# syzhang092218-source/dgppo

Hardware: AMD Instinct MI355X
Metric: env-steps/sec whole node, LidarSpread n=8 4096 envs, 1/2/4/8 GPUs (higher is better)
Workload: dtype f32

## Files before the change

dgppo_amd/csrc/env_step.h:

```cpp
#pragma once
#include "common.h"

enum { MODE_STEP = 0, MODE_SENSE = 1, MODE_GRAPH = 2 };

struct StepArgs {
  dgppo_env_cfg cfg;
  const float* agent;
  const float* action;
  const float* goal;
  const float* obst;
  const float* hits;
  const float* ray_cos;
  const float* ray_sin;
  float* next_agent;
  float* next_hits;
  float* reward;
  float* cost;
  dgppo_graph_out g;
  int has_graph;
  int mode;
  uint32_t rcp_n, rcp_k, rcp_no, rcp_no4;
  int B;
  float thr2_comm, thr2_lidar;
};

template <int SD>
__device__ inline void state2feat(const float* s, float* f) {
  if constexpr (SD == 5) {
    f[0] = s[0];
    f[1] = s[1];
    f[2] = s[4] * s[2];
    f[3] = s[4] * s[3];
  } else {
    f[0] = s[0]; f[1] = s[1]; f[2] = s[2]; f[3] = s[3];
  }
}

__device__ inline float clip_action(float u) { return clampf_nan(u, -1.0f, 1.0f); }


template <int SD>
__device__ inline void step_state(const float* x, float u0, float u1, const dgppo_env_cfg& c, float y_limit, float* nx) {
  const float dt = c.dt, A = c.area_size;
  if constexpr (SD == 5) {
    const float theta = atan2f(x[3], x[2]);
    const float theta_next = theta + x[4] * u0 * dt * 10.0f;
    nx[0] = clampf_nan(x[0] + x[4] * cosf(theta) * dt, 0.0f, A);
    nx[1] = clampf_nan(x[1] + x[4] * sinf(theta) * dt, 0.0f, A);
    nx[2] = clampf_nan(cosf(theta_next), -1.0f, 1.0f);
    nx[3] = clampf_nan(sinf(theta_next), -1.0f, 1.0f);
    nx[SD - 1] = clampf_nan(x[SD - 1] + u1 * dt * 10.0f, -0.5f, 0.5f);
  } else {
    const float vl = c.vel_limit;
    nx[0] = clampf_nan(x[2] * dt + x[0], 0.0f, A);
    nx[1] = clampf_nan(x[3] * dt + x[1], 0.0f, y_limit);
    nx[2] = clampf_nan((u0 * 10.0f) * dt + x[2], -vl, vl);
    nx[3] = clampf_nan((u1 * 10.0f) * dt + x[3], -vl, vl);
  }
}

__device__ inline float cost_value(float m) { return (m <= 0.0f) ? m - 0.5f : m + 0.5f; }

__device__ inline float reward_from_sums(float s1, float s2, float s3, int ng, int n) {
  float r = 0.0f;
  r = r - (s1 / (float)ng) * 0.01f;
  r = r - (s2 / (float)ng) * 0.001f;
  r = r - (s3 / (float)n) * 0.0001f;
  return r;
}

__device__ inline float segment_alpha_literal(float det0, float na, float nb) {
  const float sgn = (det0 > 0.0f) ? 1.0f : ((det0 < 0.0f) ? -1.0f : det0);
  const float det = sgn * fminf(fmaxf(fabsf(det0), 1e-7f), 1e7f);
  const float aq = na / det, bq = nb / det;
  const float v = ((aq <= 1.0f) && (aq >= 0.0f) && (bq <= 1.0f) && (bq >= 0.0f)) ? 1.0f : 0.0f;
  return v * aq + (1.0f - v) * 1e6f;
}

__device__ inline bool rect_inside(const float* rec, float px, float py, float r) {
  float rel_x = px - rec[0];
  float rel_y = py - rec[1];
  float c = rec[5], s = rec[6];
  float rel_xx = fabsf(rel_x * c + rel_y * s) - rec[2] / 2.0f;
  float rel_yy = fabsf(rel_x * s - rel_y * c) - rec[3] / 2.0f;
  bool is_in_down = (rel_xx < r) && (rel_yy < 0.0f);
  bool is_in_up = (rel_xx < 0.0f) && (rel_yy < r);
  bool is_out_corner = (rel_xx > 0.0f) && (rel_yy > 0.0f);
  bool is_in_circle = sqrtf(rel_xx * rel_xx + rel_yy * rel_yy) < r;
  return is_in_down || is_in_up || (is_out_corner && is_in_circle);
}


__device__ inline void segment_consts(const float* rec, int m, float* out4) {
  const int mm = (m + 3) & 3;
  const float* P = rec + 8;
  out4[0] = P[2 * m];
  out4[1] = P[2 * m + 1];
  out4[2] = P[2 * mm] - P[2 * m];
  out4[3] = P[2 * mm + 1] - P[2 * m + 1];
}

__device__ inline float ray_min_alpha(float x1, float y1, float rc, float rs, float sr, const float* s_seg, int no) {
  const float x2 = x1 + rc * sr;
  const float y2 = y1 + rs * sr;
  const float dx12 = x1 - x2, dy12 = y1 - y2;
  float amin = 0.0f;
  for (int o = 0; o < no; ++o) {
    float ao = 0.0f;
#pragma unroll
    for (int m = 0; m < 4; ++m) {
      const float4 sg = reinterpret_cast<const float4*>(s_seg)[o * 4 + m];
      const float x3 = sg.x, y3 = sg.y, ex = sg.z, ey = sg.w;
      const float det0 = dx12 * ey - dy12 * ex;
      const float ax = x1 - x3, ay = y1 - y3;
      const float na = ey * ax - ex * ay;
      const float nb = (-dy12) * ax + dx12 * ay;
      float al;
      if (det0 != 0.0f && det0 == det0) {
        const float det = copysignf(fminf(fmaxf(fabsf(det0), 1e-7f), 1e7f), det0);
        const bool pos = det > 0.0f;
        const bool va = (na == 0.0f || (na > 0.0f) == pos) && (pos ? (na <= det) : (na >= det));
        const bool vb = (nb == 0.0f || (nb > 0.0f) == pos) && (pos ? (nb <= det) : (nb >= det));
        al = 1e6f;
        if (va && vb) al = na / det + 0.0f;
      } else {
        al = segment_alpha_literal(det0, na, nb);
      }
      ao = (m == 0) ? al : nanmin(ao, al);
    }
    amin = (o == 0) ? ao : nanmin(amin, ao);
  }
  return amin;
}

__device__ inline int ray_rank(const float* al, int R, int r) {
  const float ar = al[r];
  const bool nr = (ar != ar);
  int rank = 0;
  for (int j = 0; j < R; ++j) {
    const float aj = al[j];
    const bool nj = (aj != aj);
    bool less;
    if (nj || nr) less = (nj == nr) ? (j < r) : nr;
    else less = (aj < ar) || (aj == ar && j < r);
    rank += less ? 1 : 0;
  }
  return rank;
}

__device__ inline void ray_hit(float x1, float y1, float rc, float rs, float sr, float ar, float* out2) {
  const float x2 = x1 + rc * sr;
  const float y2 = y1 + rs * sr;
  out2[0] = x1 + (x2 - x1) * ar;
  out2[1] = y1 + (y2 - y1) * ar;
}


#define MISS_BITS 0x49742400u

bool lidar_wave_has_instance(const dgppo_env_cfg& c);
void launch_lidar_wave(const StepArgs& a, hipStream_t s);
```

dgppo_amd/csrc/env_step.hip:

```cpp
#include "env_step.h"

template <int SD>
__global__ void env_step_kernel(StepArgs a) {
  extern __shared__ float smem[];
  const dgppo_env_cfg& c = a.cfg;
  const int b = blockIdx.x;
  const int tid = threadIdx.x, nt = blockDim.x;
  const int n = c.n_agents, ng = c.n_goals, no = c.n_obs, R = c.n_rays, k = c.top_k;
  const bool lidar = cfg_is_lidar(c), spread = cfg_is_spread(c);
  const int ostride = lidar ? DGPPO_RECT_STRIDE : SD;
  const int n_on = cfg_obs_nodes(c);
  const int kk = lidar ? (no > 0 ? k : 0) : 0;
  constexpr int ND = SD + 3;

  float* s_seg = smem;
  float* s_agent = s_seg + (lidar ? no * 16 : 0);
  float* s_next = s_agent + n * SD;
  float* s_goal = s_next + n * SD;
  float* s_act = s_goal + ng * SD;
  float* s_obst = s_act + n * 2;
  float* s_hpre = s_obst + no * ostride;
  float* s_hnext = s_hpre + n * kk * 2;
  float* s_alpha = s_hnext + n * kk * 2;
  float* s_fa = s_alpha + (lidar ? n * R : 0);
// ... 540 lines not shown
        const int e3 = e - n_aa - n_ag;
        i = DIVK(e3);
        const float lx = s_next[i * SD] - s_hnext[e3 * 2], ly = s_next[i * SD + 1] - s_hnext[e3 * 2 + 1];
        f = make_float4(lx, ly, 0.0f, 0.0f);
        mask = sqrtf(lx * lx + ly * ly) < c.lidar_mask_radius;
        sender = 2 * n + e3;
      }
      edges[e] = f;
      recv[e] = mask ? i : pad;
      send[e] = mask ? sender : pad;
    }
    int32_t* nty = a.g.node_type + (size_t)b * N;
    for (int node = tid; node < N; node += nt) nty[node] = (node < n) ? 0 : ((node < 2 * n) ? 1 : ((node < pad) ? 2 : -1));
    if (tid == 0) { a.g.n_node[b] = N; a.g.n_edge[b] = E; }
  }
  LDS_BARRIER();
  {
    float* nodes = a.g.nodes + (size_t)b * N * ND;
    for (int idx = tid; idx < N * ND; idx += nt) nodes[idx] = s_outn[idx];
    float* states = a.g.states + (size_t)b * N * SD;
    for (int idx = tid; idx < N * SD; idx += nt) states[idx] = s_outs[idx];
  }
}
#undef DIVN
#undef DIVK
#undef DIVNO
#undef DIVNO4

static size_t lidar_smem_bytes(const dgppo_env_cfg& c) {
  const size_t n = c.n_agents, no = c.n_obs, R = 32, k = c.top_k, SD = c.state_dim, NR = n * R;
  const size_t N = 2 * n + n * k + 1;
  size_t w = no * 16 + n * no * 16 + NR + n * 8 + no * 16 + n * SD * 3 + n * 2 + n * k * 4 + (2 * n * n + n * k) + n * no + 2 * n +
             N * (SD + 3) + N * SD;
  return w * 4;
}

static size_t step_smem_bytes(const dgppo_env_cfg& c) {
  const int n = c.n_agents, ng = c.n_goals, no = c.n_obs, SD = c.state_dim;
  const bool lidar = cfg_is_lidar(c);
  const int kk = lidar ? (no > 0 ? c.top_k : 0) : 0;
  size_t fl = (lidar ? (size_t)no * 16 : 0) + (size_t)n * SD * 2 + (size_t)ng * SD + n * 2 + (size_t)no * cfg_obst_stride(c) + (size_t)n * kk * 4 +
              (lidar ? (size_t)n * c.n_rays : 0) + n * 4 + ng * 4 + 3 * (size_t)cfg_reward_goals(c) + 3 * n + (size_t)n * no +
              (size_t)n * n + (size_t)n * (kk > no ? kk : no) + (size_t)cfg_reward_goals(c) * n;
  return fl * sizeof(float);
}

static float sqrt_threshold(float c) {
  if (!(c > 0.0f)) return 0.0f;
  float s = c * c;
  while (s > 0.0f && sqrtf(s) >= c) s = nextafterf(s, 0.0f);
  while (!(sqrtf(s) >= c)) s = nextafterf(s, INFINITY);
  return s;
}

enum StepFamily { FAMILY_WAVE, FAMILY_LIDAR_WG, FAMILY_GENERIC };

static StepFamily step_family(const StepArgs& a) {
  const dgppo_env_cfg& c = a.cfg;
  const bool lidar32 = cfg_is_lidar(c) && cfg_is_base_kind(c) && c.n_obs > 0 && c.n_rays == 32;
  auto al16 = [](const void* p) { return p == nullptr || (((uintptr_t)p) & 15) == 0; };
  const bool aligned = al16(a.agent) && al16(a.goal) && al16(a.obst) && al16(a.hits) && al16(a.next_agent) &&
                       al16(a.next_hits) && al16(a.action) && (!a.has_graph || (al16(a.g.edges) && al16(a.g.states)));
  if (lidar32 && c.top_k == 8 && c.eye_offset >= c.comm_radius && aligned && lidar_wave_has_instance(c)) return FAMILY_WAVE;
  if (lidar32 && lidar_smem_bytes(c) <= 60 * 1024) return FAMILY_LIDAR_WG;
  return FAMILY_GENERIC;
}

static int32_t launch_step(const dgppo_env_cfg* cfg, int mode, const float* agent, const float* action, const float* goal,
                           const float* obst, const float* hits, const float* ray_cos, const float* ray_sin,
                           float* next_agent, float* next_hits, float* reward, float* cost, const dgppo_graph_out* gout,
                           int32_t B, void* stream) {
  int32_t rc = dgppo_validate_cfg(cfg);
  if (rc) return rc;
  if (mode == MODE_GRAPH) DGPPO_REFUSE_VMAS(cfg, "dgppo_graph_materialize", "dgppo_vmas_graph_materialize");
  else DGPPO_REFUSE_VMAS(cfg, "dgppo_env_step", "dgppo_vmas_step");
  DGPPO_REQUIRE(B >= 0, "B must be >= 0 (got %d)", B);
  if (B == 0) return 0;
  const bool lidar = cfg_is_lidar(*cfg);
  DGPPO_REQUIRE(agent && goal, "agent/goal must not be NULL");
  DGPPO_REQUIRE(cfg->n_obs == 0 || obst, "obst must not be NULL when n_obs > 0");
  if (mode == MODE_STEP) {
    DGPPO_REQUIRE(action && reward && cost && next_agent, "step needs action, reward, cost and next_agent");
    DGPPO_REQUIRE(!(lidar && cfg->n_obs > 0) || hits, "LiDAR step needs the hit points of the current graph");
  }
  if (mode != MODE_GRAPH && lidar && cfg->n_obs > 0) {
    DGPPO_REQUIRE(ray_cos && ray_sin, "LiDAR sensing needs the ray tables");
    DGPPO_REQUIRE(next_hits || gout, "LiDAR sensing needs next_hits or a graph output");
  }
  if (mode == MODE_GRAPH) {
    DGPPO_REQUIRE(gout, "materialize needs a graph output");
    DGPPO_REQUIRE(!(lidar && cfg->n_obs > 0) || hits, "materialize needs hits for LiDAR envs");
  }
  StepArgs a;
  a.cfg = *cfg;
  a.agent = agent; a.action = action; a.goal = goal; a.obst = obst; a.hits = hits;
  a.ray_cos = ray_cos; a.ray_sin = ray_sin;
  a.next_agent = next_agent; a.next_hits = next_hits; a.reward = reward; a.cost = cost;
  a.has_graph = 0;
  a.g = dgppo_graph_out{};
  if (gout) {
    DGPPO_REQUIRE(gout->nodes && gout->edges && gout->states && gout->receivers && gout->senders && gout->node_type &&
                      gout->n_node && gout->n_edge,
                  "graph output must have all eight pointers set");
    DGPPO_REQUIRE(((uintptr_t)gout->edges & 15) == 0, "graph edges must be 16-byte aligned");
    a.g = *gout;
    a.has_graph = 1;
  }
  a.mode = mode;
  a.B = B;
  a.rcp_n = fdiv_rcp(cfg->n_agents); a.rcp_k = fdiv_rcp(cfg->top_k); a.rcp_no = fdiv_rcp(cfg->n_obs);
  a.rcp_no4 = fdiv_rcp(4 * (cfg->n_obs > 0 ? cfg->n_obs : 1));
  a.thr2_comm = sqrt_threshold(cfg->comm_radius);
  a.thr2_lidar = sqrt_threshold(cfg->lidar_mask_radius);
  const size_t smem = step_smem_bytes(*cfg);
  DGPPO_REQUIRE(smem <= 64 * 1024, "env too large for the per-env LDS stage (%zu bytes)", smem);
  hipStream_t s = (hipStream_t)stream;
  switch (step_family(a)) {
    case FAMILY_WAVE:
      launch_lidar_wave(a, s);
      break;
    case FAMILY_LIDAR_WG: {
      const size_t fsmem = lidar_smem_bytes(*cfg);
      if (cfg->state_dim == 5) hipLaunchKernelGGL((lidar_step_kernel<5, false, 128>), dim3(B), dim3(128), fsmem, s, a);
      else if (cfg_is_spread(*cfg)) hipLaunchKernelGGL((lidar_step_kernel<4, true, 128>), dim3(B), dim3(128), fsmem, s, a);
      else hipLaunchKernelGGL((lidar_step_kernel<4, false, 128>), dim3(B), dim3(128), fsmem, s, a);
      break;
    }
    case FAMILY_GENERIC: {
      int work = cfg->n_agents * (lidar ? cfg->n_rays : 1);
      const int E = cfg_num_edges(*cfg);
      if (gout && E > work) work = E;
      int threads = ((work + 63) / 64) * 64;
      if (threads < 64) threads = 64;
      if (threads > 512) threads = 512;
      if (cfg->state_dim == 5) hipLaunchKernelGGL(env_step_kernel<5>, dim3(B), dim3(threads), smem, s, a);
      else hipLaunchKernelGGL(env_step_kernel<4>, dim3(B), dim3(threads), smem, s, a);
      break;
    }
  }
  DGPPO_LAUNCH_CHECK();
  return 0;
}

extern "C" int32_t dgppo_env_step(const dgppo_env_cfg* cfg, const float* agent, const float* action, const float* goal,
                                  const float* obst, const float* hits, const float* ray_cos, const float* ray_sin,
                                  float* next_agent, float* next_hits, float* reward, float* cost,
                                  const dgppo_graph_out* gout, int32_t B, void* stream) {
  if (!cfg) { dgppo_set_error("cfg is NULL"); return -1; }
  const int mode = action ? MODE_STEP : MODE_SENSE;
  return launch_step(cfg, mode, agent, action, goal, obst, hits, ray_cos, ray_sin, next_agent, next_hits, reward, cost,
                     gout, B, stream);
}

extern "C" int32_t dgppo_graph_materialize(const dgppo_env_cfg* cfg, const float* agent, const float* goal,
                                           const float* obst, const float* hits, const dgppo_graph_out* gout, int32_t B,
                                           void* stream) {
  if (!cfg) { dgppo_set_error("cfg is NULL"); return -1; }
  return launch_step(cfg, MODE_GRAPH, agent, nullptr, goal, obst, hits, nullptr, nullptr, nullptr, nullptr, nullptr, nullptr,
                     gout, B, stream);
}
```

dgppo_amd/csrc/env_wave.hip:

```cpp
#include "env_step.h"

#ifndef DGPPO_WAVE_WPE
#define DGPPO_WAVE_WPE 5
#endif
#ifndef DGPPO_WAVE_WPE_COMPACT
#define DGPPO_WAVE_WPE_COMPACT 6
#endif
#ifndef DGPPO_WAVE_UNROLL_O
#define DGPPO_WAVE_UNROLL_O 8
#endif
#ifndef DGPPO_WAVE_UNROLL_P3
#define DGPPO_WAVE_UNROLL_P3 1
#endif
#define DGPPO_PRAGMA_(x) _Pragma(#x)
#define DGPPO_PRAGMA(x) DGPPO_PRAGMA_(x)

namespace {

#define WSYNC() asm volatile("" ::: "memory")
#ifdef DGPPO_STAMPS
__device__ unsigned long long g_wstamps[64];
__device__ unsigned long long g_wspan[3 * 8192];
#define PHASE(name, idx) do { asm volatile("; PHASE " name ::: "memory"); \
    if (blockIdx.x == 0 && threadIdx.x == 0 && stamp_on) g_wstamps[idx] = __builtin_amdgcn_s_memtime(); } while (0)
#elif defined(DGPPO_PHASE_MARKS)
#define PHASE(name, idx) asm volatile("; PHASE " name)
#else
#define PHASE(name, idx) do { } while (0)
#endif

constexpr int ceil4(int x) { return (x + 3) / 4 * 4; }

template <int SD, bool SPREAD, int NA, int NO>
struct WC {
  static constexpr int K = 8, R = 32, ND = SD + 3;
  static constexpr int NR = NA * R, NIT = NR / 64;
  static constexpr int NHIT = NA * K;
  static constexpr int N = 2 * NA + NHIT + 1, PAD = N - 1;
  static constexpr int GS = SPREAD ? NA : 1;
  static constexpr int E = NA * (NA + GS + K);
  static constexpr int NPAIR = NA * NO;
  static constexpr int NFAR = (NPAIR + 63) / 64;
  static_assert(NA % 2 == 0 && NA >= 2 && NA <= 16, "wave kernel: even n_agents <= 16 (two agents share a wave iteration)");
  static_assert((NA & (NA - 1)) == 0 && NA >= 4, "wave kernel: n_agents must be a power of two >= 4 (DPP group reductions)");
  static_assert(NO >= 1 && NO * 4 <= 64, "wave kernel: 1 <= n_obs <= 16");
  static_assert((NA * SD) % 4 == 0, "agent / goal rows are staged as float4");
  static_assert(ceil4(3 * NA) <= NA * SD && 4 * NA + ceil4(NA * 2) <= NO * 16, "overlays exceed the staged input they reuse");
};

template <int SD, bool SPREAD, int NA, int NO, bool GRAPH>
struct alignas(16) WaveLds {
  using C = WC<SD, SPREAD, NA, NO>;
  float4 seg[NO * 4];
  float4 pc[NA * NO];
  float4 circ[NO];
  uint32_t alpha[NA * 32];
  uint32_t badm[ceil4(NA)];
  union {
    uint16_t items[NA * NO * 32];
    struct {
      uint32_t tk[NA * 32];
      uint32_t hcnt[ceil4(NA)];
      uint16_t hlist[NA * 32];
    };
  };
  float next[ceil4(NA * SD)];
  union {
    float agent[NA * SD];
    float red[ceil4(3 * NA)];
  };
  float goal[NA * SD];
  union {
    float obst[NO * 16];
    struct {
      float sq[4 * NA];
      float cost[ceil4(NA * 2)];
    };
  };
  float hits[NA * C::K * 2];
  float act[ceil4(NA * 2)];
  float fa[SD == 4 ? 4 : NA * 4];
  float fg[SD == 4 ? 4 : NA * 4];
  float ino[ceil4(NA * NO)];
  float nodes[GRAPH ? ceil4(C::N * C::ND) : 4];
};

__device__ inline float raw_min(float a, float b) { float r; asm("v_min_f32 %0, %1, %2" : "=v"(r) : "v"(a), "v"(b)); return r; }
__device__ inline float raw_max(float a, float b) { float r; asm("v_max_f32 %0, %1, %2" : "=v"(r) : "v"(a), "v"(b)); return r; }

__device__ inline bool rect_inside_r0(const float* rec, float px, float py) {
  const float rel_x = px - rec[0], rel_y = py - rec[1];
  const float cs = rec[5], sn = rec[6];
  const float rel_xx = fabsf(rel_x * cs + rel_y * sn) - rec[2] / 2.0f;
  const float rel_yy = fabsf(rel_x * sn - rel_y * cs) - rec[3] / 2.0f;
  return (rel_xx < 0.0f) && (rel_yy < 0.0f);
}

template <int CTRL>
__device__ inline float dpp(float x) {
  return __int_as_float(__builtin_amdgcn_update_dpp(0, __float_as_int(x), CTRL, 0xF, 0xF, false));
}
constexpr int DPP_XOR1 = 0xB1;
constexpr int DPP_XOR2 = 0x4E;
constexpr int DPP_HALF_MIRROR = 0x141;
constexpr int DPP_ROW_MIRROR = 0x140;

template <int G>
__device__ inline float group_min(float x) {
  if (__builtin_amdgcn_ballot_w64(x != x) == 0ull) {
    x = raw_min(x, dpp<DPP_XOR1>(x));
    x = raw_min(x, dpp<DPP_XOR2>(x));
    if constexpr (G >= 8) x = raw_min(x, dpp<DPP_HALF_MIRROR>(x));
    if constexpr (G >= 16) x = raw_min(x, dpp<DPP_ROW_MIRROR>(x));
  } else {
    x = nanmin(x, dpp<DPP_XOR1>(x));
    x = nanmin(x, dpp<DPP_XOR2>(x));
    if constexpr (G >= 8) x = nanmin(x, dpp<DPP_HALF_MIRROR>(x));
    if constexpr (G >= 16) x = nanmin(x, dpp<DPP_ROW_MIRROR>(x));
  }
  return x;
}

template <int SD, bool SPREAD, int NA, int NO, int WPB, int MODE, bool GRAPH>
__global__ void __launch_bounds__(WPB * 64) __attribute__((amdgpu_waves_per_eu(GRAPH ? DGPPO_WAVE_WPE : DGPPO_WAVE_WPE_COMPACT, 8))) lidar_wave_kernel(StepArgs a) {
  using C = WC<SD, SPREAD, NA, NO>;
  using LT = WaveLds<SD, SPREAD, NA, NO, GRAPH>;
  constexpr int K = C::K, ND = C::ND, N = C::N, PAD = C::PAD, NIT = C::NIT, GS = C::GS, E = C::E;
  extern __shared__ float4 smem4[];
  int lane = threadIdx.x & 63;
  const int wave = __builtin_amdgcn_readfirstlane((int)(threadIdx.x >> 6));
  LT& L = reinterpret_cast<LT*>(smem4)[wave];
#ifdef DGPPO_STAMPS
  const int gw = blockIdx.x * WPB + wave;
  if ((threadIdx.x & 63) == 0 && gw < 8192) g_wspan[3 * gw] = __builtin_amdgcn_s_memtime();
#endif
  const dgppo_env_cfg& c = a.cfg;
  constexpr bool do_dyn = (MODE == MODE_STEP);
  constexpr bool do_sense = (MODE != MODE_GRAPH);
  constexpr bool has_graph = GRAPH;
  const float sr = c.comm_radius;
  const int r = lane & 31;
  const int hi_half = lane >> 5;
  const float cr = do_sense ? a.ray_cos[r] : 0.0f, sn = do_sense ? a.ray_sin[r] : 0.0f;
  const uint32_t below = (1u << r) - 1u;

  constexpr int I_AG = NA * SD / 4, I_OB = NO * 4, I_HI = (MODE != MODE_SENSE) ? NA * K * 2 / 4 : 0,
                I_AC = (MODE == MODE_STEP) ? NA * 2 / 4 : 0;
  constexpr int IT = 2 * I_AG + I_OB + I_HI + I_AC, NSLOT = (IT + 63) / 64;
  static_assert(MODE != MODE_STEP || (NA * 2) % 4 == 0, "the action block is staged as float4");
  const char* gsrc[NSLOT];
  uint32_t gstride[NSLOT];
  float4 pf[NSLOT];
#pragma unroll
  for (int j = 0; j < NSLOT; ++j) {
    const int q = j * 64 + lane;
    const char* base = reinterpret_cast<const char*>(a.agent);
    uint32_t stride = NA * SD * 4;
    int q0 = 0;
    if (q >= I_AG) { base = reinterpret_cast<const char*>(a.goal); q0 = I_AG; }
    if (q >= 2 * I_AG) { base = reinterpret_cast<const char*>(a.obst); stride = NO * 64; q0 = 2 * I_AG; }
    if (I_HI > 0 && q >= 2 * I_AG + I_OB) { base = reinterpret_cast<const char*>(a.hits); stride = NA * K * 8; q0 = 2 * I_AG + I_OB; }
    if (I_AC > 0 && q >= 2 * I_AG + I_OB + I_HI) { base = reinterpret_cast<const char*>(a.action); stride = NA * 8; q0 = 2 * I_AG + I_OB + I_HI; }
    gsrc[j] = base + (q - q0) * 16;
    gstride[j] = stride;
  }
  {
    const int b0 = blockIdx.x * WPB + wave;
    if (b0 < a.B) {
#pragma unroll
      for (int j = 0; j < NSLOT; ++j)
        if (j * 64 + lane < IT) pf[j] = *reinterpret_cast<const float4*>(gsrc[j] + (size_t)b0 * gstride[j]);
    }
  }
  if (has_graph)
    for (int i = lane; i < ceil4(N * ND) / 4; i += 64) reinterpret_cast<float4*>(L.nodes)[i] = make_float4(0.0f, 0.0f, 0.0f, 0.0f);
  WSYNC();
  if (has_graph)
    for (int node = lane; node < PAD; node += 64)
      L.nodes[node * ND + ((node < NA) ? SD + 2 : ((node < 2 * NA) ? SD + 1 : SD))] = 1.0f;
  WSYNC();

  for (int b = blockIdx.x * WPB + wave; b < a.B; b += gridDim.x * WPB) {
    asm volatile("" : "+v"(lane));
#ifdef DGPPO_STAMPS
    const bool stamp_on = (b == 0);
    if ((threadIdx.x & 63) == 0 && gw < 8192 && b == gw) g_wspan[3 * gw + 1] = __builtin_amdgcn_s_memtime();
    if (blockIdx.x == 0 && threadIdx.x == 0 && stamp_on) g_wstamps[40] = __builtin_amdgcn_s_memrealtime();
#endif
    PHASE("P0_stage", 0);
#pragma unroll
    for (int j = 0; j < NSLOT; ++j)
      if (j * 64 + lane < IT) reinterpret_cast<float4*>(L.agent)[j * 64 + lane] = pf[j];
    {
      const int bn = b + gridDim.x * WPB;
      if (bn < a.B) {
#pragma unroll
        for (int j = 0; j < NSLOT; ++j)
          if (j * 64 + lane < IT) pf[j] = *reinterpret_cast<const float4*>(gsrc[j] + (size_t)bn * gstride[j]);
      }
    }
    WSYNC();
    PHASE("P1a_dyn_seg_circ", 1);
    float asq = 0.0f;
    if (lane < NA) {
      const int i = lane;
      const float* x = L.agent + i * SD;
      float nx[SD];
      if (do_dyn) {
        const float u0 = clip_action(L.act[i * 2]), u1 = clip_action(L.act[i * 2 + 1]);
        step_state<SD>(x, u0, u1, c, c.area_size, nx);
        asq = u0 * u0 + u1 * u1;
      } else {
#pragma unroll
        for (int d = 0; d < SD; ++d) nx[d] = x[d];
      }
#pragma unroll
      for (int d = 0; d < SD; ++d) L.next[i * SD + d] = nx[d];
      if constexpr (SD != 4) state2feat<SD>(nx, L.fa + i * 4);
    }
    if constexpr (SD != 4)
      if (lane >= 32 && lane < 32 + NA) state2feat<SD>(L.goal + (lane - 32) * SD, L.fg + (lane - 32) * 4);
    const float* fa_ptr = (SD == 4) ? L.next : L.fa;
    const float* fg_ptr = (SD == 4) ? L.goal : L.fg;
    uint32_t robust_bits = 0;
    if (do_sense) {
      if (lane < NO * 4) {
        const int o = lane >> 2, m = lane & 3, mm = (m + 3) & 3;
        const float* P = L.obst + o * 16 + 8;
        L.seg[lane] = make_float4(P[2 * m], P[2 * m + 1], P[2 * mm] - P[2 * m], P[2 * mm + 1] - P[2 * m + 1]);
      }
      if (lane < NO) {
        const float* P = L.obst + lane * 16 + 8;
        const float cx = ((P[0] + P[2]) + (P[4] + P[6])) * 0.25f, cy = ((P[1] + P[3]) + (P[5] + P[7])) * 0.25f;
        float h2 = 0.0f;
#pragma unroll
        for (int m = 0; m < 4; ++m) {
          const float dx = P[2 * m] - cx, dy = P[2 * m + 1] - cy;
          h2 = fmaxf(h2, dx * dx + dy * dy);
        }
        const float hm = sqrtf(h2) + 0.05f, thr = sr + hm;
        L.circ[lane] = make_float4(cx, cy, thr * thr, hm);
      }
#pragma unroll
      for (int o = 0; o < NO; ++o) {
        const int m = hi_half, mm = (m + 3) & 3;
        const float* P = L.obst + o * 16 + 8;
        const float ex = P[2 * mm] - P[2 * m], ey = P[2 * mm + 1] - P[2 * m + 1];
        const float cc = cr * ey - sn * ex;
        const bool weak = !(fabsf(cc) >= 4e-4f);
        if (__builtin_amdgcn_ballot_w64(weak) == 0ull) robust_bits |= (1u << o);
      }
    }
    WSYNC();
    PHASE("P1b_far_as", 2);
    uint64_t far[C::NFAR];
    if (do_sense) {
#pragma unroll
      for (int w = 0; w < C::NFAR; ++w) {
        const int q = w * 64 + lane;
        bool isfar = false;
        if (q < C::NPAIR) {
          const int i = q / NO, o = q - i * NO;
          const float px = L.next[i * SD], py = L.next[i * SD + 1];
          L.ino[q] = rect_inside_r0(L.obst + o * 16, px, py) ? 1.0f : 0.0f;
          const float4 cc = L.circ[o];
          const float dx = px - cc.x, dy = py - cc.y;
          const bool robust = (robust_bits >> o) & 1u;
          isfar = (dx * dx + dy * dy > cc.z) && robust;
          L.pc[q] = make_float4(cc.x - px, cc.y - py, isfar ? -1.0f : (robust ? cc.w : __builtin_inff()), 0.0f);
        }
        far[w] = __builtin_amdgcn_ballot_w64(isfar);
      }
    } else {
#pragma unroll
      for (int w = 0; w < C::NFAR; ++w) far[w] = 0ull;
    }
    PHASE("P1c_cost_terms", 3);
    if (do_dyn) {
      WSYNC();
      if (lane < NA) L.sq[3 * NA + lane] = asq;
    }
    if (do_dyn) {
#pragma unroll
      for (int q0 = 0; q0 < NA * NA; q0 += 64) {
        const int q = q0 + lane, i = q / NA, j = q - i * NA;
        float d = __builtin_inff();
        if (q < NA * NA && j != i) {
          const float dx = L.agent[i * SD] - L.agent[j * SD], dy = L.agent[i * SD + 1] - L.agent[j * SD + 1];
          d = dx * dx + dy * dy;
        }
        const float md2 = group_min<NA>(d);
        if (q < NA * NA && j == 0) L.sq[i] = md2;
      }
#pragma unroll
      for (int q0 = 0; q0 < NA * K; q0 += 64) {
        const int q = q0 + lane, i = q / K;
        float d = __builtin_inff();
        if (q < NA * K) {
          const float dx = L.hits[q * 2] - L.agent[i * SD], dy = L.hits[q * 2 + 1] - L.agent[i * SD + 1];
          d = dx * dx + dy * dy;
        }
        const float mo2 = group_min<K>(d);
        if (q < NA * K && (q & (K - 1)) == 0) L.sq[NA + i] = mo2;
      }
      if constexpr (SPREAD) {
#pragma unroll
        for (int q0 = 0; q0 < NA * NA; q0 += 64) {
          const int q = q0 + lane, g = q / NA, j = q - g * NA;
          float d = __builtin_inff();
          if (q < NA * NA) {
            const float dx = L.goal[g * SD] - L.agent[j * SD], dy = L.goal[g * SD + 1] - L.agent[j * SD + 1];
            d = dx * dx + dy * dy;
          }
          const float g2 = group_min<NA>(d);
          if (q < NA * NA && j == 0) L.sq[2 * NA + g] = g2;
        }
      } else {
        if (lane < NA) {
          const int g = lane;
          const float dx = L.goal[g * SD] - L.agent[g * SD], dy = L.goal[g * SD + 1] - L.agent[g * SD + 1];
          L.sq[2 * NA + g] = dx * dx + dy * dy;
        }
      }
      WSYNC();
      static_assert(4 * NA <= 64, "one lane per pending square root");
      if (lane < 4 * NA) {
        const float rt = sqrtf(L.sq[lane]);
        const int kind = lane / NA, i = lane - kind * NA;
        if (kind == 0) {
          const float md = nanmin(rt, 1e6f);
          L.cost[i * 2] = clampf_nan(cost_value(c.two_car_radius - md), -1.0f, 1.0f);
        } else if (kind == 1) {
          L.cost[i * 2 + 1] = clampf_nan(cost_value(c.car_radius - rt), -1.0f, 1.0f);
        } else if (kind == 2) {
          L.red[i] = rt;
          L.red[NA + i] = (rt > c.dist2goal) ? 1.0f : 0.0f;
        } else {
          L.red[2 * NA + i] = rt * rt;
        }
      }
    }
    WSYNC();
    PHASE("P1d_reward", 4);
    if (do_dyn) {
      float s = 0.0f;
      if (lane < 3) {
        s = L.red[lane * NA];
#pragma unroll
        for (int g = 1; g < NA; ++g) s = s + L.red[lane * NA + g];
      }
      const float s1 = __int_as_float(__builtin_amdgcn_readlane(__float_as_int(s), 0));
      const float s2 = __int_as_float(__builtin_amdgcn_readlane(__float_as_int(s), 1));
      const float s3 = __int_as_float(__builtin_amdgcn_readlane(__float_as_int(s), 2));
      if (lane == 0) a.reward[b] = reward_from_sums(s1, s2, s3, NA, NA);
      if (lane < NA * 2) a.cost[(size_t)b * NA * 2 + lane] = L.cost[lane];
    }
    if (a.next_agent != nullptr) {
      float4* o4 = reinterpret_cast<float4*>(a.next_agent + (size_t)b * NA * SD);
      for (int i = lane; i < NA * SD / 4; i += 64) o4[i] = reinterpret_cast<const float4*>(L.next)[i];
    }
    if (has_graph) {
      for (int q = lane; q < NA * SD; q += 64) {
        const int node = q / SD, d = q - node * SD;
        const float va = L.next[q], vg = L.goal[q];
        L.nodes[node * ND + d] = va;
        L.nodes[(NA + node) * ND + d] = vg;
      }
    }
    if (has_graph) {
      float4* edges = reinterpret_cast<float4*>(a.g.edges) + (size_t)b * E;
      int32_t* recv = a.g.receivers + (size_t)b * E;
      int32_t* send = a.g.senders + (size_t)b * E;
#pragma unroll
      for (int q0 = 0; q0 < NA * NA; q0 += 64) {
        const int q = q0 + lane;
        if (q < NA * NA) {
          const int i = q / NA, j = q - i * NA;
          const float4 fi = reinterpret_cast<const float4*>(fa_ptr)[i], fj = reinterpret_cast<const float4*>(fa_ptr)[j];
          const float dx = L.next[i * SD] - L.next[j * SD], dy = L.next[i * SD + 1] - L.next[j * SD + 1];
          const bool mask = (i != j) && (dx * dx + dy * dy < a.thr2_comm);
          edges[q] = make_float4(fi.x - fj.x, fi.y - fj.y, fi.z - fj.z, fi.w - fj.w);
          recv[q] = mask ? i : PAD;
          send[q] = mask ? j : PAD;
        }
      }
#pragma unroll
      for (int q0 = 0; q0 < NA * GS; q0 += 64) {
        const int q = q0 + lane;
        if (q < NA * GS) {
          const int i = SPREAD ? q / NA : q, g = SPREAD ? q - i * NA : q;
          const float4 fi = reinterpret_cast<const float4*>(fa_ptr)[i], fg = reinterpret_cast<const float4*>(fg_ptr)[g];
          edges[NA * NA + q] = make_float4(fi.x - fg.x, fi.y - fg.y, fi.z - fg.z, fi.w - fg.w);
          recv[NA * NA + q] = i;
          send[NA * NA + q] = NA + g;
        }
      }
      int32_t* nty = a.g.node_type + (size_t)b * N;
#pragma unroll
      for (int q0 = 0; q0 < N; q0 += 64) {
        const int node = q0 + lane;
        if (node < N) nty[node] = (node < NA) ? 0 : ((node < 2 * NA) ? 1 : ((node < PAD) ? 2 : -1));
      }
      if (lane == 0) { a.g.n_node[b] = N; a.g.n_edge[b] = E; }
    }
    PHASE("P2_rays", 5);
    if (do_sense) {
      for (int q = lane; q < NA * 32 / 4; q += 64)
        reinterpret_cast<uint4*>(L.alpha)[q] = make_uint4(MISS_BITS, MISS_BITS, MISS_BITS, MISS_BITS);
      if (lane < ceil4(NA)) L.badm[lane] = 0u;
      int total = 0;
      constexpr int GSTEPS = (2 * NO * NIT <= 32) ? NIT : ((32 / (2 * NO)) >= 1 ? (32 / (2 * NO)) : 1);
      static_assert(2 * NO <= 32, "one step's triples must fit the lane mask");
#pragma unroll
      for (int g0 = 0; g0 < NIT; g0 += GSTEPS) {
        uint32_t nmask = 0u;
#pragma unroll
        for (int it = g0; it < g0 + GSTEPS && it < NIT; ++it) {
#pragma unroll
          for (int o = 0; o < NO; ++o) {
            const int qa = (it * 2) * NO + o, qb = (it * 2 + 1) * NO + o;
            const bool fa_ = (far[qa >> 6] >> (qa & 63)) & 1ull, fb_ = (far[qb >> 6] >> (qb & 63)) & 1ull;
            if (fa_ && fb_) continue;
            const float4 pc = L.pc[(it * 2 + hi_half) * NO + o];
            const float cross = cr * pc.y - sn * pc.x, dot = cr * pc.x + sn * pc.y;
            const bool need = !(fabsf(cross) > pc.z) && !(dot < -pc.z);
            nmask |= need ? (1u << ((it - g0) * 2 * NO + o)) : 0u;
          }
        }
        const int cnt = __popc(nmask);
        int inc = cnt;
        inc += __builtin_amdgcn_update_dpp(0, inc, 0x111, 0xF, 0xF, false);
        inc += __builtin_amdgcn_update_dpp(0, inc, 0x112, 0xF, 0xF, false);
        inc += __builtin_amdgcn_update_dpp(0, inc, 0x114, 0xF, 0xF, false);
        inc += __builtin_amdgcn_update_dpp(0, inc, 0x118, 0xF, 0xF, false);
        inc += __builtin_amdgcn_update_dpp(0, inc, 0x142, 0xA, 0xF, false);
        inc += __builtin_amdgcn_update_dpp(0, inc, 0x143, 0xC, 0xF, false);
        int pos = total + inc - cnt;
        total += __builtin_amdgcn_readlane(inc, 63);
        const uint32_t base_code = ((uint32_t)((2 * g0 + hi_half) * NO) << 5) | (uint32_t)r;
        while (__builtin_amdgcn_ballot_w64(nmask != 0u) != 0ull) {
          if (nmask != 0u) {
            const int bit = __builtin_ctz(nmask);
            L.items[pos] = (uint16_t)(base_code + ((uint32_t)bit << 5));
            pos += 1;
            nmask &= nmask - 1u;
          }
        }
      }
      WSYNC();
      PHASE("P2b_dense", 6);
#pragma unroll 1
      for (int k0 = 0; k0 < total; k0 += 64) {
        const int k = k0 + lane;
        const uint32_t item = L.items[k < total ? k : 0];
        const int rr = (int)(item & 31u);
        const float crr = __int_as_float(__builtin_amdgcn_ds_bpermute(rr << 2, __float_as_int(cr)));
        const float snr = __int_as_float(__builtin_amdgcn_ds_bpermute(rr << 2, __float_as_int(sn)));
        if (k < total) {
          const int pair = (int)(item >> 5);
          const int i = pair / NO, o = pair - i * NO;
          const float x1 = L.next[i * SD], y1 = L.next[i * SD + 1];
          const float x2 = x1 + crr * sr, y2 = y1 + snr * sr;
          const float dx12 = x1 - x2, dy12 = y1 - y2, ndy12 = -dy12;
          float naf[4], adet[4];
          bool valid[4];
          float dprod = 1.0f;
#pragma unroll
          for (int m = 0; m < 4; ++m) {
            const float4 sg = L.seg[o * 4 + m];
            const float ax = x1 - sg.x, ay = y1 - sg.y;
            const float na = sg.w * ax - sg.z * ay;
            const float det0 = dx12 * sg.w - dy12 * sg.z;
            const float nb = ndy12 * ax + dx12 * ay;
            const uint32_t sb = __float_as_uint(det0) & 0x80000000u;
            naf[m] = __uint_as_float(__float_as_uint(na) ^ sb);
            const float nbf = __uint_as_float(__float_as_uint(nb) ^ sb);
            adet[m] = __builtin_amdgcn_fmed3f(fabsf(det0), 1e-7f, 1e7f);
            const float mn = raw_min(naf[m], nbf), mx = raw_max(naf[m], nbf);
            valid[m] = (mn >= 0.0f) && (mx <= adet[m]);
            dprod = dprod * det0;
          }
          const bool bad = !(fabsf(dprod) > 0.0f);
          float amin = 1e6f;
          if (__builtin_amdgcn_ballot_w64(valid[0] || valid[1] || valid[2] || valid[3]) != 0ull) {
#pragma unroll
            for (int m = 0; m < 4; ++m) {
              const float qa_ = naf[m] / adet[m] + 0.0f;
              const float al = valid[m] ? qa_ : 1e6f;
              amin = raw_min(amin, al);
            }
          }
          if (amin < 1e6f) atomicMin(&L.alpha[i * 32 + rr], __float_as_uint(amin));
          if (bad) atomicOr(&L.badm[i], 1u << rr);
        }
      }
      WSYNC();
      PHASE("P2_slowcheck", 10);
      if (__builtin_amdgcn_ballot_w64(lane < NA && L.badm[lane < NA ? lane : 0] != 0u) != 0ull) {
#pragma unroll 1
        for (int it = 0; it < NIT; ++it) {
          const int i = it * 2 + hi_half;
          if ((L.badm[i] >> r) & 1u) {
            const float x1 = L.next[i * SD], y1 = L.next[i * SD + 1];
            const float x2 = x1 + cr * sr, y2 = y1 + sn * sr;
            const float dx12 = x1 - x2, dy12 = y1 - y2, ndy12 = -dy12;
            float lmin = 1e6f;
            bool any_nan = false;
#pragma unroll 1
            for (int q = 0; q < NO * 4; ++q) {
              const float4 sgq = L.seg[q];
              const float ax = x1 - sgq.x, ay = y1 - sgq.y;
              const float na = sgq.w * ax - sgq.z * ay;
// ... 58 lines not shown
          const int rr = (int)(rec & 31u);
          const float crr = __int_as_float(__builtin_amdgcn_ds_bpermute(rr << 2, __float_as_int(cr)));
          const float snr = __int_as_float(__builtin_amdgcn_ds_bpermute(rr << 2, __float_as_int(sn)));
          if (k < n_hits) {
            const int i = (int)(rec >> 10), p = (int)((rec >> 5) & 31u);
            const uint32_t kr = L.tk[i * 32 + p];
            int rank = 0;
#pragma unroll 1
            for (int cb = 0; cb < cmaxw; cb += 4) {
              const uint4 ks = *reinterpret_cast<const uint4*>(&L.tk[i * 32 + cb]);
              rank += ((ks.x < kr) || (ks.x == kr && cb + 0 < p)) ? 1 : 0;
              rank += ((ks.y < kr) || (ks.y == kr && cb + 1 < p)) ? 1 : 0;
              rank += ((ks.z < kr) || (ks.z == kr && cb + 2 < p)) ? 1 : 0;
              rank += ((ks.w < kr) || (ks.w == kr && cb + 3 < p)) ? 1 : 0;
            }
            if (rank < K) {
              const float x1 = L.next[i * SD], y1 = L.next[i * SD + 1];
              const float x2 = x1 + crr * sr, y2 = y1 + snr * sr;
              const float ar = __uint_as_float(kr);
              const float hx = x1 + (x2 - x1) * ar, hy = y1 + (y2 - y1) * ar;
              const int hq = i * K + rank, node = 2 * NA + hq;
              L.hits[hq * 2] = hx; L.hits[hq * 2 + 1] = hy;
              if (has_graph) { L.nodes[node * ND] = hx; L.nodes[node * ND + 1] = hy; }
            }
          }
        }
      } else {
        WSYNC();
  #pragma unroll 1
        for (int it = 0; it < NIT; ++it) {
          const int i = it * 2 + hi_half;
          const float x1 = L.next[i * SD], y1 = L.next[i * SD + 1];
          const float x2 = x1 + cr * sr, y2 = y1 + sn * sr;
          float is_in = 0.0f;
  #pragma unroll
          for (int o = 0; o < NO; ++o) is_in = fmaxf(is_in, L.ino[i * NO + o]);
          float ar = __uint_as_float(L.alpha[i * 32 + r]);
          ar = ar * (1.0f - is_in);
          PHASE("P3_topk", 12 + it * 3 + 1);
          int rank;
          if (__builtin_amdgcn_ballot_w64(ar != ar) == 0ull) {
            const uint32_t kr = __float_as_uint(ar);
            const bool hit = kr < MISS_BITS;
            const uint64_t Lm = __builtin_amdgcn_ballot_w64(hit);
            const uint32_t lo = (uint32_t)Lm, hi = (uint32_t)(Lm >> 32);
            const int n_lo = __popc(lo), n_hi = __popc(hi);
            const int p = (int)__builtin_amdgcn_mbcnt_hi(hi, __builtin_amdgcn_mbcnt_lo(lo, 0u)) - (hi_half ? n_lo : 0);
            const bool allz = is_in != 0.0f;
            const bool z_lo = __builtin_amdgcn_readlane((int)allz, 0) != 0, z_hi = __builtin_amdgcn_readlane((int)allz, 32) != 0;
            const int c_lo = z_lo ? 0 : n_lo, c_hi = z_hi ? 0 : n_hi;
            const int cmax = c_lo > c_hi ? c_lo : c_hi;
            rank = allz ? r : ((hi_half ? n_hi : n_lo) + r - p);
            if (cmax > 0) {
              const bool isL = hit && !allz;
              L.tk[lane] = 0xFFFFFFFFu;
              WSYNC();
              if (isL) L.tk[hi_half * 32 + p] = kr;
              WSYNC();
              int rlt = 0;
  #pragma unroll 1
              for (int cb = 0; cb < cmax; cb += 4) {
                const uint4 ks = *reinterpret_cast<const uint4*>(&L.tk[hi_half * 32 + cb]);
                rlt += (ks.x < kr ? 1 : 0) + (ks.y < kr ? 1 : 0) + (ks.z < kr ? 1 : 0) + (ks.w < kr ? 1 : 0);
              }
              WSYNC();
              if (isL) L.tk[hi_half * 32 + rlt] = (uint32_t)p;
              WSYNC();
              const bool lost = isL && (L.tk[hi_half * 32 + rlt] != (uint32_t)p);
              if (__builtin_amdgcn_ballot_w64(lost) != 0ull) {
                WSYNC();
                L.tk[lane] = 0xFFFFFFFFu;
                WSYNC();
                if (isL) L.tk[hi_half * 32 + p] = kr;
                WSYNC();
                rlt = 0;
  #pragma unroll 1
                for (int sl = 0; sl < cmax; ++sl) {
                  const uint32_t kj = L.tk[hi_half * 32 + sl];
                  rlt += (kj < kr || (kj == kr && sl < p)) ? 1 : 0;
                }
                WSYNC();
              }
              if (isL) rank = rlt;
            }
          } else {
            const uint32_t kr = (ar != ar) ? 0xFFFFFFFFu : __float_as_uint(ar);
            const uint64_t Lm = __builtin_amdgcn_ballot_w64(kr < MISS_BITS);
            const uint64_t Mm = __builtin_amdgcn_ballot_w64(kr == MISS_BITS);
            const uint64_t Zm = __builtin_amdgcn_ballot_w64(kr == 0u);
            const uint32_t lo = (uint32_t)Lm, hi = (uint32_t)(Lm >> 32);
            const uint32_t myL = hi_half ? hi : lo;
            const uint32_t myM = hi_half ? (uint32_t)(Mm >> 32) : (uint32_t)Mm;
            const int cntL = __popc(myL);
            const int rank_other = (kr == MISS_BITS) ? cntL + __popc(myM & below)
                                                     : cntL + __popc(myM) + __popc(~(myL | myM) & below);
            const bool z_lo = ((uint32_t)Zm == 0xFFFFFFFFu), z_hi = ((uint32_t)(Zm >> 32) == 0xFFFFFFFFu);
            const bool allz = hi_half ? z_hi : z_lo;
            const bool isL = (kr < MISS_BITS) && !allz;
            const int p = __popc(myL & below);
            L.tk[lane] = 0xFFFFFFFFu;
            WSYNC();
            if (isL) L.tk[hi_half * 32 + p] = kr;
            WSYNC();
            const int c_lo = z_lo ? 0 : __popc(lo), c_hi = z_hi ? 0 : __popc(hi);
            const int cmax = c_lo > c_hi ? c_lo : c_hi;
            int rlt = 0;
    #pragma unroll 1
            for (int cb = 0; cb < cmax; cb += 4) {
              const uint4 ks = *reinterpret_cast<const uint4*>(&L.tk[hi_half * 32 + cb]);
              rlt += (ks.x < kr ? 1 : 0) + (ks.y < kr ? 1 : 0) + (ks.z < kr ? 1 : 0) + (ks.w < kr ? 1 : 0);
            }
            WSYNC();
            if (isL) L.tk[hi_half * 32 + rlt] = (uint32_t)p;
            WSYNC();
            const bool lost = isL && (L.tk[hi_half * 32 + rlt] != (uint32_t)p);
            if (__builtin_amdgcn_ballot_w64(lost) != 0ull) {
              WSYNC();
              L.tk[lane] = 0xFFFFFFFFu;
              WSYNC();
              if (isL) L.tk[hi_half * 32 + p] = kr;
              WSYNC();
              rlt = 0;
    #pragma unroll 1
              for (int sl = 0; sl < cmax; ++sl) {
                const uint32_t kj = L.tk[hi_half * 32 + sl];
                rlt += (kj < kr || (kj == kr && sl < p)) ? 1 : 0;
              }
              WSYNC();
            }
            rank = allz ? r : (isL ? rlt : rank_other);
          }
          if (rank < K) {
            const float hx = x1 + (x2 - x1) * ar, hy = y1 + (y2 - y1) * ar;
            const int hq = i * K + rank, node = 2 * NA + hq;
            L.hits[hq * 2] = hx; L.hits[hq * 2 + 1] = hy;
            if (has_graph) { L.nodes[node * ND] = hx; L.nodes[node * ND + 1] = hy; }
          }
          PHASE("P3_end", 12 + it * 3 + 2);
        }
      }
    } else {
      for (int q = lane; q < NA * K; q += 64) {
        const float hx = L.hits[q * 2], hy = L.hits[q * 2 + 1];
        const int node = 2 * NA + q;
        if (has_graph) { L.nodes[node * ND] = hx; L.nodes[node * ND + 1] = hy; }
      }
    }
    WSYNC();
    PHASE("P4_compact", 7);
    if (a.next_hits != nullptr) {
      float4* o4 = reinterpret_cast<float4*>(a.next_hits + (size_t)b * NA * K * 2);
      for (int i = lane; i < NA * K * 2 / 4; i += 64) o4[i] = reinterpret_cast<const float4*>(L.hits)[i];
    }
    if (!has_graph) continue;
    PHASE("P5_graph", 8);
    {
      float4* edges = reinterpret_cast<float4*>(a.g.edges) + (size_t)b * E;
      int32_t* recv = a.g.receivers + (size_t)b * E;
      int32_t* send = a.g.senders + (size_t)b * E;
#pragma unroll
      for (int q0 = 0; q0 < NA * K; q0 += 64) {
        const int q = q0 + lane;
        if (q < NA * K) {
          const int i = q / K;
          const float lx = L.next[i * SD] - L.hits[q * 2], ly = L.next[i * SD + 1] - L.hits[q * 2 + 1];
          const bool mask = lx * lx + ly * ly < a.thr2_lidar;
          edges[NA * NA + NA * GS + q] = make_float4(lx, ly, 0.0f, 0.0f);
          recv[NA * NA + NA * GS + q] = mask ? i : PAD;
          send[NA * NA + NA * GS + q] = mask ? 2 * NA + q : PAD;
        }
      }
      float* nodes = a.g.nodes + (size_t)b * N * ND;
#pragma unroll
      for (int q0 = 0; q0 < N * ND; q0 += 64) {
        const int q = q0 + lane;
        if (q < N * ND) nodes[q] = L.nodes[q];
      }
      if constexpr (SD == 4) {
        float4* st4 = reinterpret_cast<float4*>(a.g.states + (size_t)b * N * SD);
#pragma unroll
        for (int q0 = 0; q0 < N; q0 += 64) {
          const int node = q0 + lane;
          if (node < N) {
            const float* row = L.nodes + node * ND;
            st4[node] = (node == PAD) ? make_float4(-1.0f, -1.0f, -1.0f, -1.0f) : make_float4(row[0], row[1], row[2], row[3]);
          }
        }
      } else {
        float* st = a.g.states + (size_t)b * N * SD;
#pragma unroll
        for (int q0 = 0; q0 < N * SD; q0 += 64) {
          const int q = q0 + lane;
          if (q < N * SD) {
            const int node = q / SD, d = q - node * SD;
            st[q] = (node == PAD) ? -1.0f : L.nodes[node * ND + d];
          }
        }
      }
    }
    WSYNC();
    PHASE("env_end", 9);
#ifdef DGPPO_STAMPS
    if (blockIdx.x == 0 && threadIdx.x == 0 && stamp_on) g_wstamps[41] = __builtin_amdgcn_s_memrealtime();
    if ((threadIdx.x & 63) == 0 && gw < 8192) g_wspan[3 * gw + 2] = __builtin_amdgcn_s_memtime();
#endif
  }
}

template <int SD, bool SPREAD, int NA, int NO>
void launch_inst(const StepArgs& a, hipStream_t s) {
  constexpr size_t per_wave = sizeof(WaveLds<SD, SPREAD, NA, NO, true>);
  constexpr int WPB = (per_wave * 4 <= 40 * 1024) ? 4 : ((per_wave * 2 <= 52 * 1024) ? 2 : 1);
  static_assert(per_wave * WPB <= 64 * 1024, "LDS slab too large");
  constexpr size_t smem_g = per_wave * WPB, smem_c = sizeof(WaveLds<SD, SPREAD, NA, NO, false>) * WPB;
  static int per_cu_cached[3][2] = {{0, 0}, {0, 0}, {0, 0}};
  int& per_cu = per_cu_cached[a.mode][a.has_graph ? 1 : 0];
  if (per_cu == 0) {
    int n = 0;
    hipError_t e = hipErrorUnknown;
#define OCC(M_, G_) e = hipOccupancyMaxActiveBlocksPerMultiprocessor(&n, lidar_wave_kernel<SD, SPREAD, NA, NO, WPB, M_, G_>, WPB * 64, (G_) ? smem_g : smem_c)
    if (a.mode == MODE_STEP) { if (a.has_graph) OCC(MODE_STEP, true); else OCC(MODE_STEP, false); }
    else if (a.mode == MODE_SENSE) { if (a.has_graph) OCC(MODE_SENSE, true); else OCC(MODE_SENSE, false); }
    else OCC(MODE_GRAPH, true);
#undef OCC
    per_cu = (e == hipSuccess && n > 0) ? n : 1;
  }
  int n_cu = 256;
  {
    static int cached_cu = 0;
    if (cached_cu == 0) {
      int dev = 0, v = 0;
      if (hipGetDevice(&dev) == hipSuccess && hipDeviceGetAttribute(&v, hipDeviceAttributeMultiprocessorCount, dev) == hipSuccess && v > 0)
        cached_cu = v;
      else
        cached_cu = 256;
    }
    n_cu = cached_cu;
  }
  const int max_blocks = n_cu * per_cu;
  int blocks = (a.B + WPB - 1) / WPB;
  if (blocks > max_blocks) blocks = max_blocks;
  const dim3 g(blocks), t(WPB * 64);
#define LAUNCH(M_, G_) hipLaunchKernelGGL((lidar_wave_kernel<SD, SPREAD, NA, NO, WPB, M_, G_>), g, t, (G_) ? smem_g : smem_c, s, a)
  if (a.mode == MODE_STEP) { if (a.has_graph) LAUNCH(MODE_STEP, true); else LAUNCH(MODE_STEP, false); }
  else if (a.mode == MODE_SENSE) { if (a.has_graph) LAUNCH(MODE_SENSE, true); else LAUNCH(MODE_SENSE, false); }
  else LAUNCH(MODE_GRAPH, true);
#undef LAUNCH
}

template <int SD_, bool SPREAD_, int NA_, int NO_>
struct Inst { static constexpr int SD = SD_, NA = NA_, NO = NO_; static constexpr bool SPREAD = SPREAD_; };

template <class F>
bool with_instance(const dgppo_env_cfg& c, F&& f) {
  const bool spread = cfg_is_spread(c);
  const int n = c.n_agents, no = c.n_obs, sd = c.state_dim;
#define INST(SD_, SP_, NA_, NO_) if (sd == SD_ && spread == SP_ && n == NA_ && no == NO_) { f(Inst<SD_, SP_, NA_, NO_>{}); return true; }
  INST(4, true, 8, 3);
  INST(4, false, 8, 3);
  INST(5, false, 16, 8);
  INST(4, true, 16, 8);
  INST(4, true, 4, 2);
  INST(4, false, 4, 2);
  INST(5, false, 4, 3);
#undef INST
  return false;
}

}

#ifdef DGPPO_STAMPS
extern "C" int32_t dgppo_debug_wave_stamps(unsigned long long* out) {
  return (int32_t)hipMemcpyFromSymbol(out, HIP_SYMBOL(g_wstamps), sizeof(unsigned long long) * 64);
}
extern "C" int32_t dgppo_debug_wave_spans(unsigned long long* out) {
  return (int32_t)hipMemcpyFromSymbol(out, HIP_SYMBOL(g_wspan), sizeof(unsigned long long) * 3 * 8192);
}
#endif

bool lidar_wave_has_instance(const dgppo_env_cfg& c) { return with_instance(c, [](auto) {}); }

void launch_lidar_wave(const StepArgs& a, hipStream_t s) {
  with_instance(a.cfg, [&](auto inst) {
    using I = decltype(inst);
    launch_inst<I::SD, I::SPREAD, I::NA, I::NO>(a, s);
  });
}
```

dgppo_amd/csrc/nn_elem.hip:

```cpp
#include "common.h"
#include "nn_ln.h"
#include "nn_gru.h"

using f32x4 = __attribute__((ext_vector_type(4))) float;

__device__ inline float wave_sum(float v) {
#pragma unroll
  for (int o = 32; o >= 1; o >>= 1) v += __shfl_xor(v, o);
  return v;
}
template <int NV>
__device__ inline void block_atomic_sums(const float (&v)[NV], float* dst) {
  __shared__ float s_red[4][NV];
  const int lane = threadIdx.x & 63, wave = threadIdx.x >> 6;
#pragma unroll
  for (int k = 0; k < NV; ++k) {
    const float w = wave_sum(v[k]);
    if (lane == 0) s_red[wave][k] = w;
  }
  __syncthreads();
  if (threadIdx.x < NV) {
    float t = 0.0f;
    for (int w = 0; w < (int)(blockDim.x >> 6); ++w) t += s_red[w][threadIdx.x];
    atomicAdd(dst + threadIdx.x, t);
// ... 322 lines not shown
      for (int rt = 0; rt < RTW; ++rt)
#pragma unroll
        for (int r = 0; r < 4; ++r) {
          const int rl = rt * 16 + lq * 4 + r;
          const float d = ok[rt][r] ? dh[rt][r] + du[rt][r] : 0.0f;
          const GruGateGrad gg = gru_gate_grad(d, hp[rt][r], rg[rt][r], zg[rt][r], ng[rt][r], hn[rt][r]);
          const float dar = gg.dar, daz = gg.daz, dan = gg.dan, dhn = gg.dhn;
          dh[rt][r] = d * zg[rt][r];
          if (tau > 0) {
            s_g[rl * GRU_WL + c] = dar;
            s_g[rl * GRU_WL + 64 + c] = daz;
            s_g[rl * GRU_WL + 128 + c] = dhn;
          }
          if (ok[rt][r]) {
            const size_t row = (size_t)(row0[rt][r] + tau * a.n_inner);
            float* o = a.dgi + row * 192 + c;
            o[0] = dar; o[64] = daz; o[128] = dan;
            if (DHN_ONLY) {
              a.dhn[row * GRU_H + c] = dhn;
            } else {
              float* p = a.dgh + row * 192 + c;
              p[0] = dar; p[64] = daz; p[128] = dhn;
            }
          }
        }
      if (tau == 0) break;
      GRU_LDS_BARRIER();
      fetch(tau - 1);
      __builtin_amdgcn_sched_barrier(0);
      f32x4 acc[RTW];
#pragma unroll
      for (int rt = 0; rt < RTW; ++rt) acc[rt] = f32x4{0.f, 0.f, 0.f, 0.f};
#pragma unroll
      for (int k0 = 0; k0 < 48; k0 += 16) {
        float areg[RTW][16];
#pragma unroll
        for (int rt = 0; rt < RTW; ++rt)
#pragma unroll
          for (int u = 0; u < 16; ++u) areg[rt][u] = s_g[(rt * 16 + li) * GRU_WL + (k0 + u) * 4 + lq];
        __builtin_amdgcn_sched_barrier(0);
#pragma unroll
        for (int u = 0; u < 16; ++u)
#pragma unroll
          for (int rt = 0; rt < RTW; ++rt) acc[rt] = __builtin_amdgcn_mfma_f32_16x16x4f32(areg[rt][u], breg[k0 + u], acc[rt], 0, 0, 0);
      }
#pragma unroll
      for (int rt = 0; rt < RTW; ++rt)
#pragma unroll
        for (int r = 0; r < 4; ++r) dh[rt][r] += acc[rt][r];
      cur ^= 1;
    }
    GRU_LDS_BARRIER();
  }
}

static int gru_resident(const void* fn, size_t smem) {
  int per_cu = 0, dev = 0, cus = 256;
  if (hipOccupancyMaxActiveBlocksPerMultiprocessor(&per_cu, fn, 256, smem) != hipSuccess || per_cu < 1) per_cu = 1;
  if (hipGetDevice(&dev) != hipSuccess ||
      hipDeviceGetAttribute(&cus, hipDeviceAttributeMultiprocessorCount, dev) != hipSuccess || cus < 1) cus = 256;
  return per_cu * cus;
}

static int32_t gru_check(const GruArgs& a) {
  DGPPO_REQUIRE(a.n_seq >= 0 && a.T >= 1 && a.n_inner >= 1, "gru: bad sizes n_seq=%d T=%d n_inner=%d", a.n_seq, a.T, a.n_inner);
  DGPPO_REQUIRE(a.n_seq % a.n_inner == 0, "gru: n_seq must be a multiple of n_inner");
  return 0;
}

static int32_t gru_fwd_launch(GruArgs a, hipStream_t stream) {
  int32_t rc = gru_check(a);
  if (rc) return rc;
  const int n_seq = a.n_seq;
  if (n_seq == 0) return 0;
  DGPPO_REQUIRE(a.gi && a.Wh && a.bhn && a.hs, "gru_fwd: NULL operand");
  if (cdiv(n_seq, 32) >= 512) {
    const size_t smem = sizeof(float) * 2 * 32 * GRU_HL;
    static thread_local int cap = 0;
    if (cap == 0) cap = gru_resident(reinterpret_cast<const void*>(&gru_fwd_kernel<2>), smem);
    const int tiles = cdiv(n_seq, 32);
    hipLaunchKernelGGL(gru_fwd_kernel<2>, dim3(tiles < cap ? tiles : cap), dim3(256), smem, stream, a);
  } else {
    const size_t smem = sizeof(float) * 2 * 16 * GRU_HL;
    static thread_local int cap = 0;
    if (cap == 0) cap = gru_resident(reinterpret_cast<const void*>(&gru_fwd_kernel<1>), smem);
    const int tiles = cdiv(n_seq, 16);
    hipLaunchKernelGGL(gru_fwd_kernel<1>, dim3(tiles < cap ? tiles : cap), dim3(256), smem, stream, a);
  }
  DGPPO_LAUNCH_CHECK();
  return 0;
}

extern "C" int32_t dgppo_gru_fwd(const float* gi, const float* Wh, const float* bhn, const float* h0, float* hs,
                                 float* hprev, float* gates, int32_t n_seq, int32_t T, int32_t n_inner, void* stream) {
  GruArgs a{};
  a.gi = gi; a.Wh = Wh; a.bhn = bhn; a.h0 = h0; a.hs = hs; a.hprev = hprev; a.gates = gates;
  a.n_seq = n_seq; a.T = T; a.n_inner = n_inner;
  return gru_fwd_launch(a, (hipStream_t)stream);
}

extern "C" int32_t dgppo_gru_fwd_h0_blocks(const float* gi, const float* Wh, const float* bhn, const float* h0,
                                           int32_t rows_per_block, int64_t block_stride, float* hs, float* hprev,
                                           float* gates, int32_t n_seq, int32_t T, int32_t n_inner, void* stream) {
  GruArgs a{};
  a.gi = gi; a.Wh = Wh; a.bhn = bhn; a.h0 = h0; a.hs = hs; a.hprev = hprev; a.gates = gates;
  a.n_seq = n_seq; a.T = T; a.n_inner = n_inner;
  DGPPO_REQUIRE(h0 != nullptr && ((uintptr_t)h0 & 15) == 0, "gru_fwd_h0_blocks: h0 must be a 16-byte aligned pointer");
  DGPPO_REQUIRE(rows_per_block >= 1, "gru_fwd_h0_blocks: rows_per_block must be >= 1 (got %d)", rows_per_block);
  DGPPO_REQUIRE(block_stride >= (int64_t)rows_per_block * GRU_H && block_stride % 4 == 0,
                "gru_fwd_h0_blocks: block_stride must be a multiple of 4 and >= rows_per_block * 64");
  a.h0_rpb = rows_per_block; a.h0_bstride = (long)block_stride;
  return gru_fwd_launch(a, (hipStream_t)stream);
}

template <bool DHN_ONLY>
static int32_t gru_bwd_launch(GruArgs a, hipStream_t stream) {
  int32_t rc = gru_check(a);
  if (rc) return rc;
  if (a.n_seq == 0) return 0;
  DGPPO_REQUIRE(a.dhs && a.Wh && a.hprev && a.gates && a.dgi && (DHN_ONLY ? a.dhn : a.dgh), "gru_bwd: NULL operand");
  if (cdiv(a.n_seq, 32) >= 512) {
    const size_t smem = sizeof(float) * 2 * 32 * GRU_WL;
    static thread_local int cap = 0;
    if (cap == 0) cap = gru_resident(reinterpret_cast<const void*>(&gru_bwd_kernel<2, DHN_ONLY>), smem);
    const int tiles = cdiv(a.n_seq, 32);
    hipLaunchKernelGGL((gru_bwd_kernel<2, DHN_ONLY>), dim3(tiles < cap ? tiles : cap), dim3(256), smem, stream, a);
  } else {
    const size_t smem = sizeof(float) * 2 * 16 * GRU_WL;
    static thread_local int cap = 0;
    if (cap == 0) cap = gru_resident(reinterpret_cast<const void*>(&gru_bwd_kernel<1, DHN_ONLY>), smem);
    const int tiles = cdiv(a.n_seq, 16);
    hipLaunchKernelGGL((gru_bwd_kernel<1, DHN_ONLY>), dim3(tiles < cap ? tiles : cap), dim3(256), smem, stream, a);
  }
  DGPPO_LAUNCH_CHECK();
  return 0;
}

extern "C" int32_t dgppo_gru_bwd(const float* dhs, const float* Wh, const float* hprev, const float* gates, float* dgi,
                                 float* dgh, int32_t n_seq, int32_t T, int32_t n_inner, void* stream) {
  GruArgs a{};
  a.dhs = dhs; a.Wh = Wh; a.hprev = (float*)hprev; a.gates = (float*)gates; a.dgi = dgi; a.dgh = dgh;
  a.n_seq = n_seq; a.T = T; a.n_inner = n_inner;
  return gru_bwd_launch<false>(a, (hipStream_t)stream);
}

extern "C" int32_t dgppo_gru_bwd_dhn(const float* dhs, const float* Wh, const float* hprev, const float* gates, float* dgi,
                                     float* dhn, int32_t n_seq, int32_t T, int32_t n_inner, void* stream) {
  GruArgs a{};
  a.dhs = dhs; a.Wh = Wh; a.hprev = (float*)hprev; a.gates = (float*)gates; a.dgi = dgi; a.dhn = dhn;
  a.n_seq = n_seq; a.T = T; a.n_inner = n_inner;
  return gru_bwd_launch<true>(a, (hipStream_t)stream);
}

#define STD_INIT_INV (-0.43275212956718856f)
#define STD_MIN 1e-5f
#define THRESH 0.999f
#define INV_THRESH 3.8002011672502f
#define LOG_EPS (-6.907755278982137f)
#define HALF_LOG_2PI 0.9189385332046727f
#define LOG2_F 0.6931471805599453f

__device__ inline float softplusf_(float x) { return (x > 20.0f) ? x : log1pf(expf(x)); }
#define NDTR_SERIES_BELOW (-10.0f)
__device__ inline float ndtr_tail_series(float z2) { return 1.0f - 1.0f / z2 + 3.0f / (z2 * z2) - 15.0f / (z2 * z2 * z2); }
__device__ inline float log_ndtrf_(float z) {
  if (z > NDTR_SERIES_BELOW) return logf(0.5f * erfcf(-z * 0.70710678118654752f));
  const float z2 = z * z;
  return -0.5f * z2 - logf(-z) - HALF_LOG_2PI + logf(ndtr_tail_series(z2));
}
__device__ inline float dlog_ndtrf_(float z) {
  if (z > NDTR_SERIES_BELOW) return 0.3989422804014327f * expf(-0.5f * z * z) / (0.5f * erfcf(-z * 0.70710678118654752f));
  return -z / ndtr_tail_series(z * z);
}
__device__ inline float tanh_fldj(float x) { return 2.0f * (LOG2_F - x - softplusf_(-2.0f * x)); }

struct HeadArgs {
  const float* ms;
  const float* eps;
  const float* action_in;
  float* action;
  float* log_pi;
  float* entropy;
  int rows, n_agents, mode;
  const float* log_pi_old;
  const float* adv;
  float* dms;
  float* stats;
  float clip_eps, coef_ent, inv_count;
};

__device__ inline float tn_log_prob_dim(float act, float mu, float sd) {
  const float ac = fminf(fmaxf(act, -THRESH), THRESH);
  if (ac <= -THRESH) return log_ndtrf_((-INV_THRESH - mu) / sd) - LOG_EPS;
  if (ac >= THRESH) return log_ndtrf_(-(INV_THRESH - mu) / sd) - LOG_EPS;
  const float x = atanhf(ac);
  const float z = (x - mu) / sd;
  return -0.5f * z * z - logf(sd) - HALF_LOG_2PI - tanh_fldj(x);
}

__global__ void __launch_bounds__(256) policy_head_kernel(HeadArgs a) {
  float acc[4] = {0.0f, 0.0f, 0.0f, 0.0f};
  const int rows_pad = (a.rows + 255) & ~255;
  for (int row_raw = blockIdx.x * blockDim.x + threadIdx.x; row_raw < rows_pad; row_raw += gridDim.x * blockDim.x) {
  const bool valid = row_raw < a.rows;
  const int row = valid ? row_raw : a.rows - 1;
  const float4 m = reinterpret_cast<const float4*>(a.ms)[row];
  const float mu[2] = {m.x, m.y};
  const float st[2] = {m.z, m.w};
  float sd[2];
  for (int d = 0; d < 2; ++d) sd[d] = softplusf_(st[d] + STD_INIT_INV) + STD_MIN;
  if (a.mode == 1) {
    if (valid) {
      a.action[row * 2] = tanhf(mu[0]);
      a.action[row * 2 + 1] = tanhf(mu[1]);
    }
    continue;
  }
  float act[2];
  if (a.mode == 0) {
    for (int d = 0; d < 2; ++d) act[d] = tanhf(mu[d] + sd[d] * a.eps[row * 2 + d]);
    if (valid) {
      a.action[row * 2] = act[0];
      a.action[row * 2 + 1] = act[1];
      a.log_pi[row] = tn_log_prob_dim(act[0], mu[0], sd[0]) + tn_log_prob_dim(act[1], mu[1], sd[1]);
    }
    continue;
  }
  act[0] = a.action_in[row * 2];
  act[1] = a.action_in[row * 2 + 1];
  const int ag = row % a.n_agents;
  float lp = 0.0f, ent = 0.0f;
  float dlp_dmu[2], dlp_dsd[2], dent_dmu[2], dent_dsd[2];
  for (int d = 0; d < 2; ++d) {
    const float ac = fminf(fmaxf(act[d], -THRESH), THRESH);
    if (ac <= -THRESH) {
      const float u = (-INV_THRESH - mu[d]) / sd[d];
      lp += log_ndtrf_(u) - LOG_EPS;
      const float r = dlog_ndtrf_(u);
      dlp_dmu[d] = -r / sd[d];
      dlp_dsd[d] = -r * u / sd[d];
    } else if (ac >= THRESH) {
      const float u = (mu[d] - INV_THRESH) / sd[d];
      lp += log_ndtrf_(u) - LOG_EPS;
      const float r = dlog_ndtrf_(u);
      dlp_dmu[d] = r / sd[d];
      dlp_dsd[d] = -r * u / sd[d];
    } else {
      const float x = atanhf(ac);
      const float z = (x - mu[d]) / sd[d];
      lp += -0.5f * z * z - logf(sd[d]) - HALF_LOG_2PI - tanh_fldj(x);
      dlp_dmu[d] = z / sd[d];
      dlp_dsd[d] = (z * z - 1.0f) / sd[d];
    }
    const float eh = a.eps[ag * 2 + d];
    const float y = mu[d] + sd[d] * eh;
    ent += 0.5f + HALF_LOG_2PI + logf(sd[d]) + tanh_fldj(y);
    const float th = tanhf(y);
    dent_dmu[d] = -2.0f * th;
    dent_dsd[d] = 1.0f / sd[d] - 2.0f * th * eh;
  }
  if (valid) {
    a.log_pi[row] = lp;
    a.entropy[row] = ent;
  }
  if (a.dms == nullptr) continue;
  const float A = a.adv[row];
  const float rho = expf(lp - a.log_pi_old[row]);
  const float l1 = -rho * A;
  const float l2 = -fminf(fmaxf(rho, 1.0f - a.clip_eps), 1.0f + a.clip_eps) * A;
  const float lsel = fmaxf(l1, l2);
  const float dl_dlp = ((l2 > l1) ? 0.0f : -rho * A) * a.inv_count;
  const float dl_dent = -a.coef_ent * a.inv_count;
  if (valid) {
    float4 o;
    const float dsd0 = dl_dlp * dlp_dsd[0] + dl_dent * dent_dsd[0];
    const float dsd1 = dl_dlp * dlp_dsd[1] + dl_dent * dent_dsd[1];
    o.x = dl_dlp * dlp_dmu[0] + dl_dent * dent_dmu[0];
    o.y = dl_dlp * dlp_dmu[1] + dl_dent * dent_dmu[1];
    o.z = dsd0 * sigmoidf_(st[0] + STD_INIT_INV);
    o.w = dsd1 * sigmoidf_(st[1] + STD_INIT_INV);
    reinterpret_cast<float4*>(a.dms)[row] = o;
  }
  if (valid) {
    acc[0] += lsel; acc[1] += ent; acc[2] += (l2 > l1) ? 1.0f : 0.0f; acc[3] += fabsf(rho - 1.0f);
  }
  }
  if (a.mode == 2 && a.dms != nullptr) block_atomic_sums<4>(acc, a.stats);
}

extern "C" int32_t dgppo_policy_head(const float* ms, const float* eps, const float* action_in, float* action,
                                     float* log_pi, float* entropy, int32_t rows, int32_t n_agents, int32_t mode,
                                     const float* log_pi_old, const float* adv, float* dms, float* stats, float clip_eps,
                                     float coef_ent, void* stream) {
  DGPPO_REQUIRE(rows >= 0 && n_agents >= 1 && mode >= 0 && mode <= 2, "policy_head: bad arguments");
  if (rows == 0) return 0;
  DGPPO_REQUIRE(ms, "policy_head: ms is NULL");
  DGPPO_REQUIRE(((uintptr_t)ms & 15) == 0, "policy_head: ms must be 16-byte aligned");
  if (mode == 0) DGPPO_REQUIRE(eps && action && log_pi, "policy_head(sample): NULL operand");
  if (mode == 1) DGPPO_REQUIRE(action, "policy_head(mode): NULL operand");
  if (mode == 2) {
    DGPPO_REQUIRE(eps && action_in && log_pi && entropy, "policy_head(eval): NULL operand");
    if (dms) DGPPO_REQUIRE(log_pi_old && adv && stats && ((uintptr_t)dms & 15) == 0, "policy_head(eval+loss): NULL operand");
  }
  HeadArgs a{};
  a.ms = ms; a.eps = eps; a.action_in = action_in; a.action = action; a.log_pi = log_pi; a.entropy = entropy;
  a.rows = rows; a.n_agents = n_agents; a.mode = mode; a.log_pi_old = log_pi_old; a.adv = adv; a.dms = dms; a.stats = stats;
  a.clip_eps = clip_eps; a.coef_ent = coef_ent; a.inv_count = 1.0f / (float)rows;
  const int blocks = cdiv(rows, 256);
  hipLaunchKernelGGL(policy_head_kernel, dim3(blocks < 512 ? blocks : 512), dim3(256), 0, (hipStream_t)stream, a);
  DGPPO_LAUNCH_CHECK();
  return 0;
}

__global__ void __launch_bounds__(256) value_loss_kernel(const float* __restrict__ v, const float* __restrict__ target,
                                                         float* __restrict__ dv, float* __restrict__ stats, int count,
                                                         float count_f) {
  float l[1] = {0.0f};
  for (int i = blockIdx.x * blockDim.x + threadIdx.x; i < count; i += gridDim.x * blockDim.x) {
    const float d = v[i] - target[i];
    dv[i] = d / count_f;
    l[0] += 0.5f * d * d;
  }
  block_atomic_sums<1>(l, stats);
}

extern "C" int32_t dgppo_value_loss(const float* v, const float* target, float* dv, float* stats, int32_t count,
                                    void* stream) {
  DGPPO_REQUIRE(count >= 0, "value_loss: count < 0");
  if (count == 0) return 0;
  DGPPO_REQUIRE(v && target && dv && stats, "value_loss: NULL operand");
  const int blocks = cdiv(count, 256);
  hipLaunchKernelGGL(value_loss_kernel, dim3(blocks < 256 ? blocks : 256), dim3(256), 0, (hipStream_t)stream, v, target, dv,
                     stats, count, (float)count);
  DGPPO_LAUNCH_CHECK();
  return 0;
}

__global__ void mean_agents_kernel(const float* __restrict__ x, float* __restrict__ y, int G, int n, int D, int backward,
                                   const float* __restrict__ relu_mask) {
  const int idx = blockIdx.x * blockDim.x + threadIdx.x;
  if (backward) {
    if (idx >= G * n * D) return;
    const int d = idx % D, g = idx / (n * D);
    const float v = (backward == 2) ? y[idx] + x[(size_t)g * D + d] : x[(size_t)g * D + d] / (float)n;
    y[idx] = (relu_mask == nullptr || relu_mask[idx] > 0.0f) ? v : 0.0f;
  } else {
    if (idx >= G * D) return;
    const int d = idx % D, g = idx / D;
    float acc = 0.0f;
    for (int i = 0; i < n; ++i) acc += x[((size_t)g * n + i) * D + d];
    y[idx] = acc / (float)n;
  }
}

extern "C" int32_t dgppo_mean_agents(const float* x, float* y, int32_t G, int32_t n, int32_t D, int32_t backward,
                                     const float* relu_mask, void* stream) {
  DGPPO_REQUIRE(G >= 0 && n >= 1 && D >= 1, "mean_agents: bad sizes");
  DGPPO_REQUIRE(backward >= 0 && backward <= 2, "mean_agents: backward must be 0, 1 or 2");
  if (G == 0) return 0;
  DGPPO_REQUIRE(x && y, "mean_agents: NULL operand");
  const long total = backward ? (long)G * n * D : (long)G * D;
  hipLaunchKernelGGL(mean_agents_kernel, dim3(cdiv(total, 256)), dim3(256), 0, (hipStream_t)stream, x, y, G, n, D, backward,
                     backward ? relu_mask : nullptr);
  DGPPO_LAUNCH_CHECK();
  return 0;
}

__global__ void relu_bwd_kernel(float* __restrict__ dy, const float* __restrict__ y, long count) {
  const long i = (long)blockIdx.x * blockDim.x + threadIdx.x;
  if (i < count && !(y[i] > 0.0f)) dy[i] = 0.0f;
}

extern "C" int32_t dgppo_relu_bwd(float* dy, const float* y, int64_t count, void* stream) {
// ... 8 lines not shown
```

dgppo_amd/engine.py:

```python
from __future__ import annotations

import dataclasses
from typing import Callable, Dict, Optional

import numpy as np
import os
import torch

from . import _native as N
from . import nets
from . import ops_algo as OA
from . import ops_env as OE
from . import ops_nn as K
from .utils import checkpoint as CK


@dataclasses.dataclass
class Hyper:
    gamma: float = 0.99
    gae_lambda: float = 0.95
    clip_eps: float = 0.25
    coef_ent: float = 1e-2
    max_grad_norm: float = 2.0
    lr_actor: float = 3e-4
    lr_Vl: float = 1e-3
    lr_Vh: float = 1e-3
    batch_size: int = 16384
    rnn_step: int = 16
    alpha: float = 10.0
    cbf_eps: float = 1e-2
    cbf_weight: float = 1.0
    cbf_schedule: bool = True
    train_steps: int = 100000
    actor_gnn_layers: int = 2
    Vl_gnn_layers: int = 2
    Vh_gnn_layers: int = 1
    use_rnn: bool = True
    use_lstm: bool = False
    rnn_layers: int = 1
    lagr_init: float = 0.78
    lr_lagr: float = 1e-7
    cost_weight: float = 0.0
    cost_schedule: bool = False


class RolloutData:

    def __init__(self, cfg: N.EnvCfg, B: int, T: int, device, stochastic: bool, carry_dim: int = nets.HID):
        n = cfg.n_agents
        self.cfg, self.B, self.T, self.stochastic = cfg, B, T, stochastic
        z = lambda *s: torch.empty(*s, device=device)
        step, env = OE.record_fields(cfg)
        self.step_tm = {k: z(T + 1, B, *shape) for k, shape in step.items()}
        self.env = {k: z(B, *shape) for k, shape in env.items()}
        self.step: Dict[str, torch.Tensor] = {}
        for k in OE.STEP_FIELDS:
            setattr(self, k + "_tm", self.step_tm.get(k))
            setattr(self, k, None)
        for k in OE.ENV_FIELDS:
            setattr(self, k, self.env.get(k))
        self.action_tm = z(T, B, n, 2)
        self.log_pi_tm = z(T, B, n) if stochastic else None
        self.rnn_tm = z(T + 1, B, n, carry_dim)
        self.reward_tm = z(T, B)
        self.cost_tm = z(T, B, n, cfg.n_cost)
        self._env_major = False
        views = {k: v.unbind(0) for k, v in self.step_tm.items()}
        self.states_tm = [OE.State({k: v[t] for k, v in views.items()}, self.env) for t in range(T + 1)]

    def finalize(self):
        if self._env_major:
            return self

        def tr(name, x):
            if x is None:
                return None
            cur = getattr(self, name, None)
            want = (x.shape[1], x.shape[0]) + tuple(x.shape[2:])
            if cur is None or tuple(cur.shape) != want:
                cur = torch.empty(want, device=x.device, dtype=x.dtype)
            cur.copy_(x.transpose(0, 1))
            return cur
        for k, v in self.step_tm.items():
            self.step[k] = tr(k, v)
            setattr(self, k, self.step[k])
        self.actions = tr("actions", self.action_tm)
        self.log_pis = tr("log_pis", self.log_pi_tm) if self.stochastic else None
        T, x = self.T, self.rnn_tm
        want = (x.shape[1], T + 2) + tuple(x.shape[2:])
        cur = getattr(self, "_rnn_em", None)
        if cur is None or tuple(cur.shape) != want:
            cur = torch.empty(want, device=x.device, dtype=x.dtype)
        cur[:, :T + 1].copy_(x.transpose(0, 1))
        self._rnn_em = cur
        self.rnn_states = self._rnn_em[:, :T] if self.stochastic else self._rnn_em[:, 1:T + 1]
        self.rewards = tr("rewards", self.reward_tm)
        self.costs = tr("costs", self.cost_tm)
        self._env_major = True
        return self


class OptState:
    def __init__(self, n: int, device):
        self.m = torch.zeros(n, device=device)
        self.v = torch.zeros(n, device=device)
        self.state = torch.zeros(N.OPT_STATE_FLOATS, device=device)


class Engine:
    def __init__(self, cfg: N.EnvCfg, hyper: Hyper, device, T: int = 128,
                 allreduce: Optional[Callable[[torch.Tensor], None]] = None, world: int = 1, prepass_graphs: int = 1 << 20,
                 use_graphs: bool = False, multi_stream: bool = False, algo: str = "dgppo", rank: int = 0):
        self.cfg, self.hp, self.device, self.T = cfg, hyper, device, T
        assert algo in ("dgppo", "informarl", "hcbfcrpo", "informarl_lagr"), algo
        self.algo = algo
        self.use_graphs = use_graphs and os.environ.get("DGPPO_HIPGRAPH", "1") != "0"
        self.multi_stream = multi_stream and os.environ.get("DGPPO_MULTI_STREAM", "1") != "0"
        self._side_streams = None
        self._ro_cache: Dict[tuple, dict] = {}
        self._upd_graph: dict = {}
        self.n_cost = cfg.n_cost
        spec = [("policy", "policy", hyper.actor_gnn_layers, 2), ("Vl", "Vl", hyper.Vl_gnn_layers, 1)]
        if algo == "dgppo":
            spec.append(("Vh", "Vh", hyper.Vh_gnn_layers, self.n_cost))
        elif algo == "informarl_lagr":
            spec.append(("Vh", "Vhg", hyper.Vh_gnn_layers, self.n_cost))
        def rnn_kw(name):
            if not hyper.use_rnn:
                return dict(rnn="none", rnn_layers=0)
            if name == "Vh" and algo == "dgppo":
                return dict(rnn="gru", rnn_layers=1)
            return dict(rnn="lstm" if hyper.use_lstm else "gru", rnn_layers=hyper.rnn_layers)
        sizes = [nets.make_layout(kind, cfg.node_dim, layers, n_out, **rnn_kw(k)).size for k, kind, layers, n_out in spec]
        offs, tot = [], 0
        for sz in sizes:
            offs.append(tot)
            tot += (sz + 3) // 4 * 4
        self.flat_grads = torch.zeros(tot + 4 * 8, device=device)
        self.n_reduced = tot + 3 * 8
        self.stats = self.flat_grads[tot:tot + 32].view(4, 8)
        built = {k: nets.Net(kind, cfg, layers, n_out, device, grads=self.flat_grads[o:o + sz], **rnn_kw(k))
                 for (k, kind, layers, n_out), o, sz in zip(spec, offs, sizes)}
        if algo == "informarl_lagr":
            self.lagr = torch.full((cfg.n_agents, self.n_cost), float(hyper.lagr_init), device=device)
            self.lagr_sums = torch.zeros(cfg.n_agents * self.n_cost, device=device)
        self.policy, self.Vl, self.Vh = built["policy"], built["Vl"], built.get("Vh")
        self.HC = self.policy.carry_dim
        self.opt = {k: OptState(net.layout.size, device) for k, net in self.nets.items()}
        self.arena = nets.Arena(device)
        self.allreduce = allreduce
        self.world, self.rank = int(world), int(rank)
        assert self.world >= 1 and (allreduce is not None or self.world == 1), "world > 1 needs an allreduce"
        assert 0 <= self.rank < self.world, f"rank {rank} outside world {world}"
        self.prepass_graphs = int(os.environ.get("DGPPO_PREPASS_GRAPHS", prepass_graphs))
        self.lam_pow = OA.lam_pow_table(hyper.gae_lambda, T, device)
        self.eps_hat = torch.zeros(cfg.n_agents, 2, device=device)
        self.reset_failed = torch.zeros(1, dtype=torch.int32, device=device)
        self.grad_hook: Optional[Callable[[str, nets.Net, int], None]] = None
        self._mb = 0

    @property
    def nets(self) -> Dict[str, nets.Net]:
        d = {"policy": self.policy, "Vl": self.Vl}
        if self.Vh is not None:
            d["Vh"] = self.Vh
        return d

    def set_entropy_noise(self, seed: int):
        OE.randn(seed, 0, self.eps_hat.view(-1))

    _CFG_IDENTITY = ("kind", "n_agents", "n_obs", "n_rays", "top_k", "node_dim", "n_cost")

    def _identity(self) -> dict:
        ident = {"algo": CK.encode_str(self.algo)}
        ident.update({f"cfg.{k}": int(getattr(self.cfg, k)) for k in self._CFG_IDENTITY})
        for f in dataclasses.fields(Hyper):
            v = getattr(self.hp, f.name)
            ident[f"hyper.{f.name}"] = int(v) if isinstance(v, (bool, int)) else float(v)
        ident["T"], ident["world"] = int(self.T), int(self.world)
        ident.update({f"size.{k}": int(net.layout.size) for k, net in self.nets.items()})
        return ident

    def _state_tensors(self) -> Dict[str, torch.Tensor]:
        t = {}
        for k, net in self.nets.items():
            opt = self.opt[k]
            t.update({f"{k}/params": net.params, f"{k}/m": opt.m, f"{k}/v": opt.v, f"{k}/state": opt.state})
        t["eps_hat"] = self.eps_hat
        if self.algo == "informarl_lagr":
            t["lagr"] = self.lagr
        return t

    def state_dict(self) -> dict:
        out = {"identity": self._identity()}
        for path, x in self._state_tensors().items():
            node = out
            *dirs, leaf = path.split("/")
            for d in dirs:
                node = node.setdefault(d, {})
            node[leaf] = x.detach().cpu().numpy().copy()
        return out

    def load_state_dict(self, d: dict) -> None:
        mine, theirs = self._identity(), d.get("identity", {})
        show = lambda v: repr(CK.decode_str(v)) if isinstance(v, np.ndarray) else repr(v)
        for k, v in mine.items():
            if k not in theirs:
                raise ValueError(f"state dict does not fit this engine: it has no identity field '{k}'")
            if not np.array_equal(np.asarray(v), np.asarray(theirs[k])):
                raise ValueError(f"state dict does not fit this engine: '{k}' is {show(theirs[k])} there, {show(v)} here")
        src = {}
        for path, x in self._state_tensors().items():
            node = d
            for part in path.split("/"):
                node = node.get(part) if isinstance(node, dict) else None
            if not isinstance(node, np.ndarray) or node.dtype != np.float32 or node.shape != tuple(x.shape):
                raise ValueError(f"state dict does not fit this engine: '{path}' is not a float32 array of shape {tuple(x.shape)}")
            src[path] = node
        for path, x in self._state_tensors().items():
            x.copy_(torch.from_numpy(src[path]).to(self.device))
        for net in self.nets.values():
            net.prepare()

    def _feats(self, tag, st: OE.State, n_env, n_time=1, slots=1, env_ids=None):
        f = nets.GraphFeats(self.cfg, n_env * n_time, self.arena, tag)
        return f.compute_record(st.step, slots, st.env, env_ids, n_env, n_time)

    def _rollout_steps(self, ro: RolloutData, eps, B: int, stochastic: bool):
        cfg, T, n = self.cfg, self.T, self.cfg.n_agents
        tag = "ro" if stochastic else "rod"
        for t in range(T):
            feats = self._feats(tag, ro.states_tm[t], B)
            act = self.policy.forward(feats, n_seq=B * n, T=1, h0=ro.rnn_tm[t].view(B * n, self.HC), tag=tag,
                                      hs_out=ro.rnn_tm[t + 1].view(B * n, self.HC), train=False)
            a_t = ro.action_tm[t].view(B * n, 2)
            if stochastic:
                K.policy_head(act["ms"], eps[t], None, a_t, ro.log_pi_tm[t].view(B * n), None, n, 0)
            else:
                K.policy_head(act["ms"], None, None, a_t, None, None, n, 1)
            OE.step(cfg, ro.states_tm[t], ro.action_tm[t], ro.states_tm[t + 1], ro.reward_tm[t], ro.cost_tm[t])

    def rollout(self, seeds: torch.Tensor, stochastic: bool, noise_seed: int = 0) -> RolloutData:
        cfg, T = self.cfg, self.T
        B = int(seeds.shape[0])
        n = cfg.n_agents
        slot = None
        if self.use_graphs:
            slot = self._ro_cache.setdefault((B, stochastic), {"ro": None, "graph": None, "gen": -1, "calls": 0})
            if slot["ro"] is None:
                slot["ro"] = RolloutData(cfg, B, T, self.device, stochastic, self.HC)
            ro = slot["ro"]
            ro._env_major = False
        else:
            ro = RolloutData(cfg, B, T, self.device, stochastic, self.HC)
        OE.reset(cfg, seeds, ro.states_tm[0], self.reset_failed)
        ro.rnn_tm[0].zero_()
        eps = None
        if stochastic:
            eps = self.arena.get("ro.eps", T, B * n, 2)
            OE.randn_rows(noise_seed, eps.view(T, B * n * 2), self.world * B * n * 2, self.rank * B * n * 2)
        if slot is None:
            self._rollout_steps(ro, eps, B, stochastic)
            return ro
        slot["calls"] += 1
        if slot["graph"] is not None and slot["gen"] != self._arena_generation():
            slot["graph"] = None
        if slot["graph"] is not None:
            slot["graph"].replay()
            K.FLOPS[0] += slot.get("flops", 0.0)
            return ro
        f0 = K.FLOPS[0]
        self._rollout_steps(ro, eps, B, stochastic)
        slot["flops"] = K.FLOPS[0] - f0
        if not slot.get("failed", False):
            graph = torch.cuda.CUDAGraph()
            try:
                f1 = K.FLOPS[0]
                with torch.cuda.graph(graph, capture_error_mode="thread_local"):
                    self._rollout_steps(ro, eps, B, stochastic)
                K.FLOPS[0] = f1 + slot["flops"]
                slot["graph"], slot["gen"] = graph, self._arena_generation()
                graph.replay()
            except Exception as ex:
                slot["failed"] = True
                torch.cuda.synchronize()
                print(f"[dgppo_amd] HIP-graph capture of the rollout loop failed ({type(ex).__name__}: {ex}); "
                      f"continuing with eager launches", flush=True)
        return ro

    def _update_generation(self) -> int:
        return self.arena.generation + sum(net.arena.generation + net.ws_arena.generation for net in self.nets.values())

    def _arena_generation(self) -> int:
        return self.arena.generation + self.policy.arena.generation

    def rollout_pair(self, seeds: torch.Tensor, det_seeds: torch.Tensor, noise_seed: int = 0):
        if not (self.multi_stream and self.device.type == "cuda"):
            return self.rollout(seeds, True, noise_seed), self.rollout(det_seeds, False)
        main = torch.cuda.current_stream(self.device)
        s0, s1 = self._net_streams()[:2]
        out = [None, None]
        for k, (st, sd, stoch) in enumerate(((s0, seeds, True), (s1, det_seeds, False))):
            st.wait_stream(main)
            with torch.cuda.stream(st):
                out[k] = self.rollout(sd, stoch, noise_seed if stoch else 0)
        main.wait_stream(s0)
        main.wait_stream(s1)
        return out[0], out[1]

    def _block_feats(self, tag, ro: RolloutData, e0, Eb, t0, n_time, env_ids=None):
        envs = slice(e0, None) if env_ids is None else slice(None)
        st = OE.State({k: v[envs, t0] for k, v in ro.step.items()}, {k: v[envs] for k, v in ro.env.items()})
        return self._feats(tag, st, Eb, n_time, self.T + 1, env_ids)

    def _vh_carry(self, ro: RolloutData, e0: int, Eb: int) -> torch.Tensor:
        return ro.rnn_states[e0:e0 + Eb][..., :nets.HID]

    def _final_carry(self, ro: RolloutData, e0: int, Eb: int) -> torch.Tensor:
        T, n, HC = self.T, self.cfg.n_agents, self.HC
        fin = self._block_feats("fin", ro, e0, Eb, T, 1)
        h_last = self.arena.get("pre.hlast", Eb * n, HC)
        h_last.view(Eb, n, HC).copy_(ro.rnn_states[e0:e0 + Eb, T - 1])
        hstar = self.arena.get("pre.hstar", Eb * n, HC)
        self.policy.forward(fin, n_seq=Eb * n, T=1, h0=h_last, tag="fin", hs_out=hstar, train=False)
        return hstar

    def values_prepass(self, ro: RolloutData, want_Vl: bool, want_Vh: bool = True):
        cfg, T, B = self.cfg, self.T, ro.B
        n, nh, H = cfg.n_agents, self.n_cost, nets.HID
        kind = "ro" if ro.stochastic else "det"
        Vl_buf = self.arena.get(f"tg.Vl.{kind}", B, T + 1) if want_Vl else None
        Vh_buf = self.arena.get(f"tg.Vh.{kind}", B, T + 1, n, nh) if want_Vh else None
        block = max(1, min(B, self.prepass_graphs // (T + 1)))
        for e0 in range(0, B, block):
            Eb = min(block, B - e0)
            feats = self._block_feats("pre", ro, e0, Eb, 0, T + 1)
            if want_Vl:
                act = self.Vl.forward(feats, n_seq=Eb, T=T + 1, h0=None, tag="pre", train=False)
                Vl_buf[e0:e0 + Eb].copy_(act["v"].view(Eb, T + 1))
            if not want_Vh:
                continue
            HC = self.HC
            hstar = self._final_carry(ro, e0, Eb)
            if not self.hp.use_rnn:
                h0 = None
            elif HC == H:
                s0 = 0 if ro.stochastic else 1
                ro._rnn_em[e0:e0 + Eb, s0 + T].copy_(hstar.view(Eb, n, H))
                h0 = K.H0Blocks(ro._rnn_em[e0, s0], (T + 1) * n, (T + 2) * n * H, Eb)
            else:
                h0_all = self.arena.get("pre.h0all", Eb, T + 1, n, H)
                h0_all[:, :T].copy_(self._vh_carry(ro, e0, Eb))
                h0_all[:, T].copy_(hstar.view(Eb, n, HC)[..., :H])
                h0 = h0_all.view(-1, H)
            act = self.Vh.forward(feats, n_seq=Eb * (T + 1) * n, T=1, h0=h0, tag="pre", train=False)
            Vh_buf[e0:e0 + Eb].copy_(act["v"].view(Eb, T + 1, n, nh))
        return Vl_buf, Vh_buf

    def require_landscape(self, what: str = "vh_landscape"):
        if self.algo != "dgppo":
            why = {"informarl_lagr": "its constraint-value net carries its own scan state, which needs a sequence pass first"}
            raise ValueError(f"{what}: algo '{self.algo}' is not supported: "
                             + why.get(self.algo, "it has no constraint-value network"))
        if self.cfg.is_vmas:
            raise ValueError(f"{what}: VMASReverseTransport is not supported")

    def vh_landscape(self, ro: RolloutData, env_index: int, agent_id: int, frame_ids, xs, ys,
                     events: Optional[list] = None) -> torch.Tensor:
        self.require_landscape()
        cfg, T = self.cfg, self.T
        n, nh, H = cfg.n_agents, self.n_cost, nets.HID
        ro.finalize()
        if not 0 <= int(env_index) < ro.B:
            raise ValueError(f"vh_landscape: env_index {env_index} outside [0, {ro.B})")
        if not 0 <= int(agent_id) < n:
            raise ValueError(f"vh_landscape: agent_id {agent_id} outside [0, {n})")
        frames = np.asarray(frame_ids, dtype=np.int64).reshape(-1)
        if frames.size == 0 or frames.min() < 0 or frames.max() >= T:
            raise ValueError(f"vh_landscape: frame_ids must be a non-empty subset of [0, {T})")
        xs, ys = K.sweep_axis(xs, "xs", self.device), K.sweep_axis(ys, "ys", self.device)
        nx, ny, F = int(xs.numel()), int(ys.numel()), int(frames.size)
        e = int(env_index)
        step = {k: v[e] for k, v in ro.step.items()}
# ... 543 lines not shown
```

dgppo_amd/nets.py:

```python
from __future__ import annotations

import math
from typing import Dict, List, Optional, Tuple

import numpy as np
import torch

from . import _native as N
from . import ops_nn as K

H_HEADS = 3
MSG_DIM = 32
OUT_DIM = 64
HID = 64


def _ceil4(x):
    return (x + 3) // 4 * 4


class Layout:
    def __init__(self):
        self.entries: Dict[str, Tuple[int, Tuple[int, ...]]] = {}
        self.size = 0
# ... 55 lines not shown

    def get(self, name: str, *shape, dtype=torch.float32, zero=False) -> torch.Tensor:
        n = math.prod(shape)
        b = self.bufs.get(name)
        if b is None or b.numel() < n or b.dtype != dtype:
            if b is not None:
                self.generation += 1
            b = torch.empty(max(n, 1), dtype=dtype, device=self.device)
            self.bufs[name] = b
        v = b[:n].view(shape)
        if zero:
            v.zero_()
        return v


class GraphFeats:

    def __init__(self, cfg: N.EnvCfg, G: int, arena: Arena, tag: str):
        self.cfg, self.G = cfg, G
        n, S = cfg.n_agents, cfg.fan_in
        self.n_other = cfg.num_nodes - 1 - n
        self.Fp = input_width(cfg)
        self.Xa = arena.get(f"{tag}.Xa0", G * n, self.Fp)
        self.Xo = arena.get(f"{tag}.Xo0", max(G * self.n_other, 1), self.Fp)[:G * self.n_other]
        self.efeat = arena.get(f"{tag}.efeat", G * n, S, 4)
        self.emask = arena.get(f"{tag}.emask", G * n, S)

    def compute(self, agent, agent_se, agent_st, goal, obst, hits, hits_se, hits_st, env_ids, n_env, n_time):
        assert n_env * n_time == self.G
        K.graph_feats(self.cfg, agent, agent_se, agent_st, goal, obst, hits, hits_se, hits_st, env_ids, n_env, n_time,
                      self.Xa, self.Xo if self.n_other > 0 else None, self.efeat, self.emask, self.Fp)
        return self

    def compute_record(self, step, slots: int, env, env_ids, n_env, n_time):
        cfg, n = self.cfg, self.cfg.n_agents
        se, st = slots, int(slots > 1)
        if cfg.is_vmas:
            return self.compute_vmas(step["agent"], se * n * 4, st * n * 4, step["body"], se * 4, st * 4, env["scene"], env_ids,
                                     n_env, n_time)
        ia, ih = n * cfg.state_dim, n * cfg.top_k * 2
        return self.compute(step["agent"], se * ia, st * ia, env["goal"], env.get("obst"), step.get("hits"), se * ih, st * ih,
                            env_ids, n_env, n_time)

    def compute_sweep(self, step, env, frame_ids, n_frames, agent_id, xs, ys, ray_cos=None, ray_sin=None, hits_out=None,
                      frame_max=None):
        cfg, n = self.cfg, self.cfg.n_agents
        if cfg.is_vmas:
            raise ValueError("compute_sweep: VMASReverseTransport has no sweep entry point")
        K.graph_feats_sweep(cfg, step["agent"], n * cfg.state_dim, env["goal"], env.get("obst"), step.get("hits"),
                            n * cfg.top_k * 2, ray_cos, ray_sin, frame_ids, n_frames, agent_id, xs, ys, self.Xa,
                            self.Xo if self.n_other > 0 else None, self.efeat, self.emask, self.Fp, hits_out, frame_max)
        return self

    def compute_action_sweep(self, step, env, frame_ids, n_frames, agent_id, us, vs, frame_max=None):
        cfg, n = self.cfg, self.cfg.n_agents
        if cfg.is_vmas:
            raise ValueError("compute_action_sweep: VMASReverseTransport has no sweep entry point")
        K.graph_feats_action_sweep(cfg, step["agent"], n * cfg.state_dim, env["goal"], env.get("obst"), step.get("hits"),
                                   n * cfg.top_k * 2, frame_ids, n_frames, agent_id, us, vs, self.Xa,
                                   self.Xo if self.n_other > 0 else None, self.efeat, self.emask, self.Fp, frame_max)
        return self

    def compute_team_action_sweep(self, st, nst, a_pol, us, vs):
        if self.cfg.is_vmas:
            raise ValueError("compute_team_action_sweep: VMASReverseTransport has no sweep entry point")
        K.graph_feats_team_action_sweep(self.cfg, st.step["agent"], nst.step["agent"], st.env["goal"], st.env.get("obst"),
                                        nst.step.get("hits"), a_pol, us, vs, self.Xa, self.Xo if self.n_other > 0 else None,
                                        self.efeat, self.emask, self.Fp)
        return self

    def compute_vmas(self, agent, agent_se, agent_st, body, body_se, body_st, scene, env_ids, n_env, n_time):
        assert n_env * n_time == self.G
        K.vmas_graph_feats(self.cfg, agent, agent_se, agent_st, body, body_se, body_st, scene, env_ids, n_env, n_time,
                           self.Xa, self.efeat, self.emask, self.Fp)
        return self


def input_width(cfg: N.EnvCfg) -> int:
    return _ceil4(cfg.node_dim) if cfg.is_vmas else 8


class Net:

    def __init__(self, kind: str, cfg: N.EnvCfg, gnn_layers: int, n_out: int, device, grads: Optional[torch.Tensor] = None,
                 rnn: str = "gru", rnn_layers: int = 1):
        assert kind in ("policy", "Vl", "Vh", "Vhg")
        self.kind, self.cfg, self.gnn_layers, self.n_out, self.device = kind, cfg, gnn_layers, n_out, device
        self.rnn, self.rnn_layers = rnn, (rnn_layers if rnn != "none" else 0)
        self.carry_dim = HID * max(self.rnn_layers, 1) * (2 if rnn == "lstm" else 1)
        self.layout = make_layout(kind, cfg.node_dim, gnn_layers, n_out, rnn, rnn_layers)
        self.params = torch.zeros(self.layout.size, device=device)
        if grads is None:
            grads = torch.zeros(self.layout.size, device=device)
        assert grads.shape == (self.layout.size,) and grads.is_contiguous() and grads.data_ptr() % 16 == 0
        self.grads = grads
        self.arena = Arena(device)
        self.ws_arena = Arena(device)
        self._views: Dict[tuple, torch.Tensor] = {}
        self.dims = []
        f = cfg.node_dim
        for l in range(gnn_layers):
            d = OUT_DIM if l == gnn_layers - 1 else MSG_DIM
            fp = input_width(cfg) if l == 0 else f
            kp = _ceil4(fp + H_HEADS * (fp + 4) + 1)
            self.dims.append((f, fp, d, kp))
            f = d
        self.prep_layout = Layout()
        for l, (f, fp, d, kp) in enumerate(self.dims):
            self.prep_layout.add(f"gnn{l}.Mcat", fp, H_HEADS * fp)
            self.prep_layout.add(f"gnn{l}.cvec", H_HEADS * fp)
            self.prep_layout.add(f"gnn{l}.Wout", kp, d)
        self.prep = torch.zeros(self.prep_layout.size, device=device)
        self.prep_grads = torch.zeros(self.prep_layout.size, device=device)

    def _cached(self, kind: str, layout, flat, name):
        key = (kind, name)
        v = self._views.get(key)
        if v is None:
            v = self._views[key] = layout.view(flat, name)
        return v

    def p(self, name):
        return self._cached("p", self.layout, self.params, name)

    def g(self, name):
        return self._cached("g", self.layout, self.grads, name)

    def pp(self, name):
        return self._cached("pp", self.prep_layout, self.prep, name)

    def pg(self, name):
        return self._cached("pg", self.prep_layout, self.prep_grads, name)

    def prepare(self):
        for l, (f, fp, d, kp) in enumerate(self.dims):
            q = lambda nm: self.p(f"gnn{l}.{nm}")
            K.gnn_prep(q("Wq"), q("bq"), q("Wk"), q("Wv"), q("bv"), q("We"), q("Wu"), self.pp(f"gnn{l}.Mcat"),
                       self.pp(f"gnn{l}.cvec"), self.pp(f"gnn{l}.Wout"), f, fp, d, H_HEADS, kp)

    def _xo_fusable(self, l: int) -> bool:
        if l != 0 or self.gnn_layers != 2:
            return False
        key = "_xo_ok"
        if not hasattr(self, key):
            f1, fp1, d1, kp1 = self.dims[1]
            setattr(self, key, self.dims[0][1] == 8 and self.dims[0][2] == 32 and fp1 == 32 and
                    K.attn_xo_supported(self.cfg, fp1, H_HEADS, kp1))
        return getattr(self, key)

    def zero_grads(self):
        self.grads.zero_()

    def forward(self, feats: GraphFeats, n_seq: int, T: int, h0: Optional[torch.Tensor], tag: str = "f",
                hs_out: Optional[torch.Tensor] = None, train: bool = True):
        cfg, G, A = self.cfg, feats.G, self.arena
        n = cfg.n_agents
        R = G * n
        Ro = G * feats.n_other
        act = {"feats": feats, "G": G, "n_seq": n_seq, "T": T}
        Xa, Xo = feats.Xa, feats.Xo
        xo_fused = None
        for l, (f, fp, d, kp) in enumerate(self.dims):
            qt = A.get(f"{tag}.qt{l}", R, H_HEADS * fp)
            K.dense_fwd(Xa, self.pp(f"gnn{l}.Mcat"), self.pp(f"gnn{l}.cvec"), qt)
            zcat = A.get(f"{tag}.zcat{l}", R, kp)
            attn = A.get(f"{tag}.attn{l}", R, cfg.fan_in, H_HEADS) if train else None
            if xo_fused is not None:
                K.attn_fwd_xo(cfg, fp, H_HEADS, kp, qt, Xa, xo_fused[0], xo_fused[1], xo_fused[2], feats.efeat, feats.emask, zcat, attn, G)
            else:
                K.attn_fwd(cfg, fp, H_HEADS, kp, qt, Xa, Xo if Ro > 0 else None, feats.efeat, feats.emask, zcat, attn, G)
            act[f"xo_fused{l}"] = xo_fused
            xo_fused = None
            Xa_n = A.get(f"{tag}.Xa{l + 1}", R, d)
            K.dense_fwd(zcat, self.pp(f"gnn{l}.Wout"), self.p(f"gnn{l}.bu"), Xa_n, act=1)
            act[f"Xa{l}"], act[f"Xo{l}"], act[f"qt{l}"], act[f"zcat{l}"], act[f"attn{l}"] = Xa, Xo, qt, zcat, attn
            if l < self.gnn_layers - 1 and Ro > 0:
                if self._xo_fusable(l):
                    xo_fused = (Xo, self.pp(f"gnn{l}.Wout")[:fp], self.p(f"gnn{l}.bu"))
                    Xo = None
                else:
                    Xo_n = A.get(f"{tag}.Xo{l + 1}", Ro, d)
                    K.dense_fwd(Xo, self.pp(f"gnn{l}.Wout")[:fp], self.p(f"gnn{l}.bu"), Xo_n, act=1)
                    Xo = Xo_n
            Xa = Xa_n
        act[f"Xa{self.gnn_layers}"] = Xa
        if self.kind == "Vl":
            pooled = A.get(f"{tag}.pool", G, OUT_DIM)
            K.mean_agents(Xa, pooled, G, n, OUT_DIM)
            x, Rh, n_inner = pooled, G, 1
        else:
            x, Rh, n_inner = Xa, R, n
        if self.kind == "Vhg":
            pooled = A.get(f"{tag}.pool", G, OUT_DIM)
            K.mean_agents(Xa, pooled, G, n, OUT_DIM)
            xcat = A.get(f"{tag}.xcat", R, 2 * OUT_DIM)
            xcat[:, :OUT_DIM].copy_(Xa)
            xcat.view(G, n, 2 * OUT_DIM)[:, :, OUT_DIM:].copy_(pooled.view(G, 1, OUT_DIM).expand(G, n, OUT_DIM))
            x = xcat
        act["Rh"], act["n_inner"], act["mlp_in"] = Rh, n_inner, x
        gi = A.get(f"{tag}.gi", Rh, 3 * HID)
        if self.kind == "Vhg" or self.rnn != "gru":
            sv = {nm: A.get(f"{tag}.{nm}", Rh, w) for nm, w in (("p1", HID), ("y1", HID), ("st1", 2), ("p2", HID), ("y2", HID), ("st2", 2))}
            K.dense_fwd(x, self.p("mlp.W1"), self.p("mlp.b1"), sv["p1"])
            K.ln_relu_fwd(sv["p1"], self.p("mlp.g1"), self.p("mlp.be1"), sv["y1"], sv["st1"])
            K.dense_fwd(sv["y1"], self.p("mlp.W2"), self.p("mlp.b2"), sv["p2"])
            K.ln_relu_fwd(sv["p2"], self.p("mlp.g2"), self.p("mlp.be2"), sv["y2"], sv["st2"])
            if self.rnn == "gru":
                K.dense_fwd(sv["y2"], self.p("gru.Wi"), self.p("gru.bi"), gi)
            act.update(sv)
        else:
            saves = None
            if train:
                saves = tuple(A.get(f"{tag}.{nm}{i}", Rh, w) for i in (1, 2) for nm, w in (("p", HID), ("y", HID), ("st", 2)))
                for i in (1, 2):
                    act[f"p{i}"], act[f"y{i}"], act[f"st{i}"] = saves[3 * (i - 1):3 * i]
            K.mlp_gi_fwd(x, self.p("mlp.W1"), self.p("mlp.b1"), self.p("mlp.g1"), self.p("mlp.be1"), self.p("mlp.W2"),
                         self.p("mlp.b2"), self.p("mlp.g2"), self.p("mlp.be2"), self.p("gru.Wi"), self.p("gru.bi"), gi, saves)
        assert n_seq * T == Rh, (n_seq, T, Rh)
        L, CD = self.rnn_layers, self.carry_dim
        h0_blocks = isinstance(h0, K.H0Blocks)
        if h0_blocks:
            assert self.rnn == "gru" and L == 1 and T == 1 and not train and self.kind != "policy", \
                "a blocked h0 serves the one-cell GRU value nets' T = 1 inference pass"
        elif h0 is not None:
            assert tuple(h0.shape) == (n_seq, CD), (tuple(h0.shape), n_seq, CD)
        if hs_out is not None:
            assert tuple(hs_out.shape) == (Rh, CD), (tuple(hs_out.shape), Rh, CD)
        act["gi"] = gi
        simple = (self.rnn == "gru" and L == 1)
        if simple:
            hs = hs_out if hs_out is not None else A.get(f"{tag}.hs", Rh, HID)
            hprev_is_h0 = train and T == 1 and h0 is not None and self.kind != "policy"
            hprev = A.get(f"{tag}.hprev", Rh, HID) if (train and not hprev_is_h0) else None
            gates = A.get(f"{tag}.gates", Rh, 4 * HID) if train else None
            feat = hs
            act["hs"], act["hprev"], act["gates"] = hs, hprev, gates
        fused_tail = (simple and T == 1 and self.kind == "policy")
        if simple and not fused_tail:
            if h0_blocks:
                K.gru_fwd_h0_blocks(gi, self.p("gru.Wh"), self.p("gru.bhn"), h0, hs, hprev, gates, n_seq, T, n_inner)
            else:
                K.gru_fwd(gi, self.p("gru.Wh"), self.p("gru.bhn"), h0, hs, hprev, gates, n_seq, T, n_inner)
            if hprev_is_h0:
                act["hprev"] = act["h0"] = h0
        if self.rnn == "none":
            feat = act["y2"]
            if hs_out is not None:
                if h0 is not None and T == 1:
                    hs_out.copy_(h0)
                else:
                    hs_out.zero_()
        elif self.rnn == "lstm":
            x_l = act["y2"]
            act["stack"] = []
            for l in range(L):
                zi = A.get(f"{tag}.zi{l}", Rh, 4 * HID)
                for half in (slice(0, 2 * HID), slice(2 * HID, 4 * HID)):
                    K.dense_fwd(x_l, self.p(f"lstm{l}.Wi")[:, half], None, zi[:, half])
                c0_l = h0_l = None
                if h0 is not None:
                    c0_l, h0_l = A.get(f"{tag}.c0_{l}", n_seq, HID), A.get(f"{tag}.h0_{l}", n_seq, HID)
                    c0_l.copy_(h0[:, (2 * l) * HID:(2 * l + 1) * HID])
                    h0_l.copy_(h0[:, (2 * l + 1) * HID:(2 * l + 2) * HID])
                cs_l, hs_l = A.get(f"{tag}.cs{l}", Rh, HID), A.get(f"{tag}.hs{l}", Rh, HID)
                cprev_l = A.get(f"{tag}.cprev{l}", Rh, HID) if train else None
                hprev_l = A.get(f"{tag}.hprev{l}", Rh, HID) if train else None
                gates_l = A.get(f"{tag}.gates{l}", Rh, 4 * HID) if train else None
                K.lstm_fwd(zi, self.p(f"lstm{l}.Wh"), self.p(f"lstm{l}.bh"), c0_l, h0_l, cs_l, hs_l, cprev_l, hprev_l, gates_l,
                           n_seq, T, n_inner)
                if hs_out is not None:
                    hs_out[:, (2 * l) * HID:(2 * l + 1) * HID].copy_(cs_l)
                    hs_out[:, (2 * l + 1) * HID:(2 * l + 2) * HID].copy_(hs_l)
                act["stack"].append(dict(x=x_l, hs=hs_l, cprev=cprev_l, hprev=hprev_l, gates=gates_l))
                x_l = hs_l
            feat = x_l
        elif not simple:
            x_l = None
            act["stack"] = []
            for l in range(L):
                pre = "gru" if l == 0 else f"gru{l}"
                gi_l = gi if l == 0 else A.get(f"{tag}.gi{l}", Rh, 3 * HID)
                if l > 0:
                    K.dense_fwd(x_l, self.p(f"{pre}.Wi"), self.p(f"{pre}.bi"), gi_l)
                h0_l = None
                if h0 is not None:
                    h0_l = A.get(f"{tag}.h0_{l}", n_seq, HID)
                    h0_l.copy_(h0[:, l * HID:(l + 1) * HID])
                hs_l = A.get(f"{tag}.hs{l}", Rh, HID)
                hprev_l = A.get(f"{tag}.hprev{l}", Rh, HID) if train else None
                gates_l = A.get(f"{tag}.gates{l}", Rh, 4 * HID) if train else None
                K.gru_fwd(gi_l, self.p(f"{pre}.Wh"), self.p(f"{pre}.bhn"), h0_l, hs_l, hprev_l, gates_l, n_seq, T, n_inner)
                if hs_out is not None:
                    hs_out[:, l * HID:(l + 1) * HID].copy_(hs_l)
                act["stack"].append(dict(x=x_l, gi=gi_l, hs=hs_l, hprev=hprev_l, gates=gates_l))
                x_l = hs_l
            feat = x_l
        act["feat"] = feat
        if self.kind == "policy":
            u = A.get(f"{tag}.u", Rh, HID) if (train or not fused_tail) else None
            ms = A.get(f"{tag}.ms", Rh, 4)
            if fused_tail:
                K.gru1_head_fwd(gi, self.p("gru.Wh"), self.p("gru.bhn"), h0, self.p("head.Ws"), self.p("head.bs"),
                                self.p("head.Wms"), self.p("head.bms"), hs, hprev, gates, u, ms)
            else:
                K.dense_fwd(feat, self.p("head.Ws"), self.p("head.bs"), u)
                K.dense_fwd(u, self.p("head.Wms"), self.p("head.bms"), ms)
            act["u"], act["ms"] = u, ms
        else:
            v = A.get(f"{tag}.v", Rh, self.n_out)
            K.dense_fwd(feat, self.p("head.Wo"), self.p("head.bo"), v)
            act["v"] = v
        return act

    def backward(self, act, dout: torch.Tensor, tag: str = "b"):
        A = self.arena
        ws_floats = getattr(self, "_bwdw_floats", 16 << 20)

# ... 252 lines not shown
```

dgppo_amd/ops_env.py:

```python
from __future__ import annotations

import ctypes as C
from typing import Dict, Optional

import numpy as np
import torch

from . import _native as N


STEP_FIELDS, ENV_FIELDS = ("agent", "hits", "body"), ("goal", "obst", "scene")


def record_fields(cfg: N.EnvCfg) -> tuple[Dict[str, tuple], Dict[str, tuple]]:
    n, sd = cfg.n_agents, cfg.state_dim
    if cfg.is_vmas:
        return {"agent": (n, 4), "body": (4,)}, {"scene": (8,)}
    step, env = {"agent": (n, sd)}, {"goal": (cfg.n_goals, sd)}
    if cfg.is_lidar and cfg.n_obs > 0:
        step["hits"] = (n, cfg.top_k, 2)
    if cfg.n_obs > 0:
        env["obst"] = (cfg.n_obs, cfg.obst_stride)
    return step, env

# ... 77 lines not shown
    go.node_type = N.ptr(g["node_type"], torch.int32, "graph.node_type")
    go.n_node = N.ptr(g["n_node"], torch.int32, "graph.n_node")
    go.n_edge = N.ptr(g["n_edge"], torch.int32, "graph.n_edge")
    return go


def _check_state(cfg: N.EnvCfg, B: int, **given):
    for fields in record_fields(cfg):
        for name, shape in fields.items():
            if given.get(name) is not None:
                N.expect_shape(given[name], (B,) + shape, name)
            elif name != "hits":
                raise ValueError(f"{name} is required by env kind {cfg.kind}")


def env_step(cfg: N.EnvCfg, agent, action, goal, obst, hits, ray_cos, ray_sin,
             next_agent, next_hits, reward, cost, graph: Optional[Dict[str, torch.Tensor]] = None):
    B = agent.shape[0]
    _check_state(cfg, B, agent=agent, goal=goal, obst=obst)
    n = cfg.n_agents
    if hits is not None:
        N.expect_shape(hits, (B, n, cfg.top_k, 2), "hits")
    if action is not None:
        N.expect_shape(action, (B, n, 2), "action")
        N.expect_shape(reward, (B,), "reward")
        N.expect_shape(cost, (B, n, cfg.n_cost), "cost")
    if next_agent is not None:
        N.expect_shape(next_agent, (B, n, cfg.state_dim), "next_agent")
    if next_hits is not None:
        N.expect_shape(next_hits, (B, n, cfg.top_k, 2), "next_hits")
    if cfg.is_lidar and cfg.n_obs > 0:
        N.expect_shape(ray_cos, (cfg.n_rays,), "ray_cos")
        N.expect_shape(ray_sin, (cfg.n_rays,), "ray_sin")
    go = _graph_out(cfg, graph, B) if graph is not None else None
    rc = N.lib().dgppo_env_step(
        C.byref(cfg), N.ptr(agent, name="agent"), N.ptr(action, name="action"), N.ptr(goal, name="goal"),
        N.ptr(obst, name="obst"), N.ptr(hits, name="hits"), N.ptr(ray_cos, name="ray_cos"), N.ptr(ray_sin, name="ray_sin"),
        N.ptr(next_agent, name="next_agent"), N.ptr(next_hits, name="next_hits"), N.ptr(reward, name="reward"),
        N.ptr(cost, name="cost"), C.byref(go) if go is not None else None, C.c_int32(B), N.stream_ptr())
    N.check(rc, "dgppo_env_step")


def graph_materialize(cfg: N.EnvCfg, agent, goal, obst, hits, graph: Dict[str, torch.Tensor]):
    B = agent.shape[0]
    _check_state(cfg, B, agent=agent, goal=goal, obst=obst)
    if hits is not None:
        N.expect_shape(hits, (B, cfg.n_agents, cfg.top_k, 2), "hits")
    go = _graph_out(cfg, graph, B)
    rc = N.lib().dgppo_graph_materialize(
        C.byref(cfg), N.ptr(agent, name="agent"), N.ptr(goal, name="goal"), N.ptr(obst, name="obst"),
        N.ptr(hits, name="hits"), C.byref(go), C.c_int32(B), N.stream_ptr())
    N.check(rc, "dgppo_graph_materialize")


def env_reset(cfg: N.EnvCfg, seeds: torch.Tensor, agent, goal, obst, n_failed: torch.Tensor = None):
    B = seeds.shape[0]
    _check_state(cfg, B, agent=agent, goal=goal, obst=obst)
    if n_failed is not None:
        N.expect_shape(n_failed, (1,), "n_failed")
    rc = N.lib().dgppo_env_reset_checked(C.byref(cfg), N.ptr(seeds, torch.int64, "seeds"), N.ptr(agent, name="agent"),
                                         N.ptr(goal, name="goal"), N.ptr(obst, name="obst"),
                                         N.ptr(n_failed, torch.int32, "n_failed"), C.c_int32(B), N.stream_ptr())
    N.check(rc, "dgppo_env_reset")


def randn_rows(seed: int, out: torch.Tensor, global_row_len: int, col_offset: int):
    rows = int(out.shape[0])
    row_len = out.numel() // max(rows, 1)
    rc = N.lib().dgppo_randn_rows(C.c_uint64(seed & 0xFFFFFFFFFFFFFFFF), N.ptr(out, name="out"), C.c_int64(rows),
                                  C.c_int64(row_len), C.c_int64(global_row_len), C.c_int64(col_offset), N.stream_ptr())
    N.check(rc, "dgppo_randn_rows")


def randn(seed: int, offset: int, out: torch.Tensor):
    rc = N.lib().dgppo_randn(C.c_uint64(seed & 0xFFFFFFFFFFFFFFFF), C.c_uint64(offset), N.ptr(out, name="out"),
                             C.c_int64(out.numel()), N.stream_ptr())
    N.check(rc, "dgppo_randn")


def _check_vmas(cfg: N.EnvCfg, agent, body, scene, B):
    if not cfg.is_vmas:
        raise ValueError(f"env kind {cfg.kind} is not VMASReverseTransport")
    _check_state(cfg, B, agent=agent, body=body, scene=scene)


def vmas_reset(cfg: N.EnvCfg, seeds: torch.Tensor, agent, body, scene, n_failed: torch.Tensor = None):
    B = seeds.shape[0]
    _check_vmas(cfg, agent, body, scene, B)
    if n_failed is not None:
        N.expect_shape(n_failed, (1,), "n_failed")
    rc = N.lib().dgppo_vmas_reset_checked(C.byref(cfg), N.ptr(seeds, torch.int64, "seeds"), N.ptr(agent, name="agent"),
                                          N.ptr(body, name="body"), N.ptr(scene, name="scene"),
                                          N.ptr(n_failed, torch.int32, "n_failed"), C.c_int32(B), N.stream_ptr())
    N.check(rc, "dgppo_vmas_reset_checked")


def vmas_step(cfg: N.EnvCfg, agent, body, scene, action, next_agent, next_body, reward, cost,
              graph: Optional[Dict[str, torch.Tensor]] = None):
    B = agent.shape[0]
    _check_vmas(cfg, agent, body, scene, B)
    n = cfg.n_agents
    N.expect_shape(action, (B, n, 2), "action")
    N.expect_shape(next_agent, (B, n, 4), "next_agent")
    N.expect_shape(next_body, (B, 4), "next_body")
    N.expect_shape(reward, (B,), "reward")
    N.expect_shape(cost, (B, n, 2), "cost")
    go = _graph_out(cfg, graph, B) if graph is not None else None
    rc = N.lib().dgppo_vmas_step(
        C.byref(cfg), N.ptr(agent, name="agent"), N.ptr(body, name="body"), N.ptr(scene, name="scene"),
        N.ptr(action, name="action"), N.ptr(next_agent, name="next_agent"), N.ptr(next_body, name="next_body"),
        N.ptr(reward, name="reward"), N.ptr(cost, name="cost"), C.byref(go) if go is not None else None, C.c_int32(B),
        N.stream_ptr())
    N.check(rc, "dgppo_vmas_step")


def vmas_graph_materialize(cfg: N.EnvCfg, agent, body, scene, graph: Dict[str, torch.Tensor]):
    B = agent.shape[0]
    _check_vmas(cfg, agent, body, scene, B)
    go = _graph_out(cfg, graph, B)
    rc = N.lib().dgppo_vmas_graph_materialize(C.byref(cfg), N.ptr(agent, name="agent"), N.ptr(body, name="body"),
                                              N.ptr(scene, name="scene"), C.byref(go), C.c_int32(B), N.stream_ptr())
    N.check(rc, "dgppo_vmas_graph_materialize")


def sense(cfg: N.EnvCfg, st: State, graph: Optional[Dict[str, torch.Tensor]] = None):
    s, e = st.step, st.env
    if "hits" not in s:
        s["hits"] = torch.empty(s["agent"].shape[:-2] + record_fields(cfg)[0]["hits"], device=s["agent"].device)
    rc, rs = _rays(cfg, s["agent"].device)
    env_step(cfg, s["agent"], None, e["goal"], e.get("obst"), None, rc, rs, None, s["hits"], None, None, graph)


def reset(cfg: N.EnvCfg, seeds: torch.Tensor, st: State, n_failed: torch.Tensor = None,
          graph: Optional[Dict[str, torch.Tensor]] = None):
    if cfg.is_vmas:
        vmas_reset(cfg, seeds, st.agent, st.body, st.scene, n_failed)
    else:
        env_reset(cfg, seeds, st.agent, st.goal, st.obst, n_failed)
    if "hits" in st.step:
        sense(cfg, st, graph)
    elif graph is not None:
        materialize(cfg, st, graph)


def step(cfg: N.EnvCfg, st: State, action, nst: State, reward, cost, graph: Optional[Dict[str, torch.Tensor]] = None):
    s, e, ns = st.step, st.env, nst.step
    if cfg.is_vmas:
        return vmas_step(cfg, s["agent"], s["body"], e["scene"], action, ns["agent"], ns["body"], reward, cost, graph)
    rc, rs = _rays(cfg, s["agent"].device)
    env_step(cfg, s["agent"], action, e["goal"], e.get("obst"), s.get("hits"), rc, rs, ns["agent"], ns.get("hits"), reward,
             cost, graph)


def materialize(cfg: N.EnvCfg, st: State, graph: Dict[str, torch.Tensor]):
    if cfg.is_vmas:
        return vmas_graph_materialize(cfg, st.agent, st.body, st.scene, graph)
    graph_materialize(cfg, st.agent, st.goal, st.obst, st.hits, graph)
```

include/dgppo_hip.h:

```cpp
#ifndef DGPPO_HIP_H
#define DGPPO_HIP_H

#include <stdint.h>

#ifdef __cplusplus
extern "C" {
#endif

#define DGPPO_ABI_VERSION 3

enum {
  DGPPO_ENV_LIDAR_SPREAD = 0,
  DGPPO_ENV_LIDAR_TARGET = 1,
  DGPPO_ENV_LIDAR_BICYCLE_TARGET = 2,
  DGPPO_ENV_MPE_SPREAD = 3,
  DGPPO_ENV_MPE_TARGET = 4,
  DGPPO_ENV_LIDAR_LINE = 5,
  DGPPO_ENV_MPE_LINE = 6,
  DGPPO_ENV_MPE_FORMATION = 7,
  DGPPO_ENV_MPE_CORRIDOR = 8,
  DGPPO_ENV_MPE_CONNECT_SPREAD = 9,
  DGPPO_ENV_VMAS_REVERSE_TRANSPORT = 10
};
enum {
  DGPPO_GOALS_NODES = 0,
  DGPPO_GOALS_LINE = 1,
  DGPPO_GOALS_LINE_INTERIOR = 2,
  DGPPO_GOALS_CIRCLE = 3
};

#define DGPPO_RECT_STRIDE 16

typedef struct dgppo_env_cfg {
  int32_t kind;
  int32_t n_agents;
  int32_t n_goals;
  int32_t n_obs;
  int32_t n_rays;
  int32_t top_k;
  int32_t state_dim;
  int32_t node_dim;
  float area_size;
  float dt;
  float car_radius;
  float comm_radius;
  float obs_radius;
  float dist2goal;
  float two_car_radius;
  float lidar_mask_radius;
  float eye_offset;
  float car_plus_obs;
  float vel_limit;
  float reset_min_dist;
  int32_t reward_goals;
  int32_t n_cost;
  float obs_mask_radius;
  float y_limit;
  float connect_radius;
  float reset_side_y;
  float goal_shift_y;
  float line_min_dist;
} dgppo_env_cfg;

typedef struct dgppo_graph_out {
  float*   nodes;
  float*   edges;
  float*   states;
  int32_t* receivers;
  int32_t* senders;
  int32_t* node_type;
  int32_t* n_node;
  int32_t* n_edge;
} dgppo_graph_out;

int32_t     dgppo_abi_version(void);
const char* dgppo_last_error(void);

int32_t dgppo_env_num_nodes(const dgppo_env_cfg* cfg);
int32_t dgppo_env_num_edges(const dgppo_env_cfg* cfg);


int32_t dgppo_env_step(const dgppo_env_cfg* cfg,
                       const float* agent, const float* action, const float* goal,
                       const float* obst, const float* hits,
                       const float* ray_cos, const float* ray_sin,
                       float* next_agent, float* next_hits, float* reward, float* cost,
                       const dgppo_graph_out* gout, int32_t B, void* stream);

int32_t dgppo_graph_materialize(const dgppo_env_cfg* cfg,
                                const float* agent, const float* goal,
                                const float* obst, const float* hits,
                                const dgppo_graph_out* gout, int32_t B, void* stream);

int32_t dgppo_env_reset(const dgppo_env_cfg* cfg, const uint64_t* seeds,
                        float* agent, float* goal, float* obst, int32_t B, void* stream);
int32_t dgppo_env_reset_checked(const dgppo_env_cfg* cfg, const uint64_t* seeds, float* agent, float* goal, float* obst,
                                int32_t* n_failed, int32_t B, void* stream);


int32_t dgppo_vmas_reset_checked(const dgppo_env_cfg* cfg, const uint64_t* seeds, float* agent, float* body, float* scene,
                                 int32_t* n_failed, int32_t B, void* stream);
int32_t dgppo_vmas_step(const dgppo_env_cfg* cfg, const float* agent, const float* body, const float* scene,
                        const float* action, float* next_agent, float* next_body, float* reward, float* cost,
                        const dgppo_graph_out* gout, int32_t B, void* stream);
int32_t dgppo_vmas_graph_materialize(const dgppo_env_cfg* cfg, const float* agent, const float* body, const float* scene,
                                     const dgppo_graph_out* gout, int32_t B, void* stream);
int32_t dgppo_vmas_graph_feats(const dgppo_env_cfg* cfg, const float* agent, int64_t agent_se, int64_t agent_st,
                               const float* body, int64_t body_se, int64_t body_st, const float* scene,
                               const int32_t* env_ids, int32_t n_env, int32_t n_time, float* Xa, float* efeat, float* emask,
                               int32_t Fp, void* stream);

int32_t dgppo_randn(uint64_t seed, uint64_t offset, float* out, int64_t n_elem, void* stream);
int32_t dgppo_randn_rows(uint64_t seed, float* out, int64_t rows, int64_t row_len, int64_t global_row_len,
                         int64_t col_offset, void* stream);


int32_t dgppo_dense_fwd(const float* X, int32_t ldx, const float* W, int32_t ldw, const float* bias, float* Y,
                        int32_t ldy, int32_t M, int32_t K, int32_t N, int32_t act, int32_t accumulate,
                        int32_t trans_w, const float* relu_mask, int32_t ldm, void* stream);
int32_t dgppo_dense_bwd_w(const float* X, int32_t ldx, const float* dY, int32_t ldy, float* dW, int32_t ldw,
                          float* db, int32_t M, int32_t K, int32_t N, float* workspace, int64_t workspace_bytes,
                          void* stream);
int32_t dgppo_mlp_gi_fwd(const float* X, int32_t ldx, const float* W1, const float* b1, const float* g1, const float* be1,
                         const float* W2, const float* b2, const float* g2, const float* be2, const float* Wi,
                         const float* bi, float* p1, float* y1, float* st1, float* p2, float* y2, float* st2, float* gi,
                         int32_t M, void* stream);
int32_t dgppo_mlp_gi_bwd(const float* dgi, const float* Wi, const float* W2, const float* W1, const float* g2,
                         const float* g1, const float* p2, const float* y2, const float* st2, const float* p1,
                         const float* y1, const float* st1, const float* relu_mask, int32_t ldm, float* dpre2, float* dpre1,
                         float* dx, int32_t lddx, float* dg2, float* db2, float* dg1, float* db1, int32_t M, void* stream);
#define DGPPO_REDUCE_BATCH 16
typedef struct dgppo_reduce_desc {
  const float* part;
  float* dW;
  float* db;
  int32_t part_stride, slabs, ldw, K, N;
  int32_t pending;
} dgppo_reduce_desc;
int32_t dgppo_dense_bwd_w_deferred(const float* X, int32_t ldx, const float* dY, int32_t ldy, float* dW, int32_t ldw,
                                   float* db, int32_t M, int32_t K, int32_t N, float* workspace, int64_t workspace_bytes,
                                   dgppo_reduce_desc* pending, void* stream);
int32_t dgppo_dense_bwd_w_reduce_batch(const dgppo_reduce_desc* descs, int32_t n, void* stream);
int32_t dgppo_dense_bwd_xw(const float* X, int32_t ldx, const float* dY, int32_t ldy, const float* W, int32_t ldw, float* dX,
                           int32_t lddx, int32_t accumulate_mask, float* dW, int32_t lddw, float* db, int32_t M, int32_t K,
                           int32_t N, float* workspace, int64_t workspace_bytes, dgppo_reduce_desc* pending, void* stream);
int64_t dgppo_mlp_gi_bwd_w_workspace_bytes(void);
int32_t dgppo_mlp_gi_bwd_w(const float* dgi, const float* Wi, const float* W2, const float* W1, const float* g2,
                           const float* g1, const float* p2, const float* y2, const float* st2, const float* p1,
                           const float* y1, const float* st1, const float* x, int32_t ldx, const float* relu_mask,
                           int32_t ldm, float* dpre2, float* dpre1, float* dx, int32_t lddx, float* dg2, float* db2,
                           float* dg1, float* db1, float* dW2, int32_t ldw2, float* dbias2, float* dW1, int32_t ldw1,
                           float* dbias1, int32_t M, float* workspace, int64_t workspace_bytes, dgppo_reduce_desc* pending,
                           void* stream);
int64_t dgppo_head_bwd_workspace_bytes(void);
int32_t dgppo_head_bwd(const float* feat, int32_t ldf, const float* u, const float* dout, const float* W1, const float* W2,
                       float* dhs, float* dW1, int32_t ldw1, float* db1, float* dW2, int32_t ldw2, float* db2, int32_t M,
                       int32_t n_out, float* workspace, int64_t workspace_bytes, dgppo_reduce_desc* pending, void* stream);
int32_t dgppo_gru1_head_fwd(const float* gi, const float* Wh, const float* bhn, const float* h0, const float* W1,
                            const float* b1, const float* W2, const float* b2, float* hs, float* hprev, float* gates,
                            float* u, float* out, int32_t M, int32_t n_out, void* stream);
int64_t dgppo_dense_bwd_w_workspace_bytes(int32_t K, int32_t N);

#define DGPPO_GATHER_MAX 8
typedef struct dgppo_gather_desc {
  const void* src;
  void* dst;
  int64_t row_bytes, src_stride;
} dgppo_gather_desc;
int32_t dgppo_gather_rows(const dgppo_gather_desc* descs, int32_t n_desc, const int32_t* ids, int32_t n_ids, void* stream);

int32_t dgppo_graph_feats(const dgppo_env_cfg* cfg, const float* agent, int64_t agent_se, int64_t agent_st,
                          const float* goal, const float* obst, const float* hits, int64_t hits_se, int64_t hits_st,
                          const int32_t* env_ids, int32_t n_env, int32_t n_time, float* Xa, float* Xo, float* efeat,
                          float* emask, int32_t Fp, void* stream);

int32_t dgppo_graph_feats_sweep(const dgppo_env_cfg* cfg, const float* agent, int64_t agent_st, const float* goal,
                                const float* obst, const float* hits, int64_t hits_st, const float* ray_cos,
                                const float* ray_sin, const int32_t* frame_ids, int32_t n_frames, int32_t agent_id,
                                const float* xs, int32_t nx, const float* ys, int32_t ny, float* Xa, float* Xo,
                                float* efeat, float* emask, float* hits_out, int32_t Fp, void* stream);

int32_t dgppo_cost_sweep(const dgppo_env_cfg* cfg, const float* agent, int64_t agent_st, const float* obst, const float* hits,
                         int64_t hits_st, const float* ray_cos, const float* ray_sin, const int32_t* frame_ids,
                         int32_t n_frames, int32_t agent_id, const float* xs, int32_t nx, const float* ys, int32_t ny,
                         float* cost, float* hits_out, void* stream);

int32_t dgppo_graph_feats_action_sweep(const dgppo_env_cfg* cfg, const float* agent, int64_t agent_st, const float* goal,
                                       const float* obst, const float* hits, int64_t hits_st, const int32_t* frame_ids,
                                       int32_t n_frames, int32_t agent_id, const float* us, int32_t nu, const float* vs,
                                       int32_t nv, float* Xa, float* Xo, float* efeat, float* emask, int32_t Fp, void* stream);

int32_t dgppo_graph_feats_team_action_sweep(const dgppo_env_cfg* cfg, const float* agent, const float* next_agent,
                                            const float* goal, const float* obst, const float* next_hits, const float* a_pol,
                                            int32_t n_env, const float* us, int32_t nu, const float* vs, int32_t nv, float* Xa,
                                            float* Xo, float* efeat, float* emask, int32_t Fp, void* stream);

int32_t dgppo_shield_select(const float* Vh_next, const float* Vh_t, const float* a_pol, int32_t n_env, int32_t n_agents,
                            int32_t n_cost, const float* us, int32_t nu, const float* vs, int32_t nv, float dt, float alpha,
                            float margin, float* action, int32_t* index, int32_t* flag, float* h, void* stream);

int32_t dgppo_attn_fwd(const dgppo_env_cfg* cfg, int32_t F, int32_t H, int32_t Kp, const float* qt, const float* Xa,
                       const float* Xo, const float* efeat, const float* emask, float* zcat, float* attn, int32_t G,
                       void* stream);
int32_t dgppo_attn_bwd(const dgppo_env_cfg* cfg, int32_t F, int32_t H, int32_t Kp, const float* dzcat,
                       const float* attn, const float* qt, const float* Xa, const float* Xo, const float* efeat,
                       float* dqt, float* dXa, float* dXo, int32_t relu_xo, int32_t G, void* stream);
int32_t dgppo_attn_xo_supported(const dgppo_env_cfg* cfg, int32_t F, int32_t H, int32_t Kp);
int32_t dgppo_attn_fwd_xo(const dgppo_env_cfg* cfg, int32_t F, int32_t H, int32_t Kp, const float* qt, const float* Xa,
                          const float* Xo_raw, const float* Wo, int32_t ldwo, const float* bo, const float* efeat,
                          const float* emask, float* zcat, float* attn, int32_t G, void* stream);
int32_t dgppo_attn_bwd_xo(const dgppo_env_cfg* cfg, int32_t F, int32_t H, int32_t Kp, const float* dzcat,
                          const float* attn, const float* qt, const float* Xa, const float* Xo_raw, const float* Wo,
                          int32_t ldwo, const float* bo, const float* efeat, float* dqt, float* dXa, float* dXo,
                          int32_t relu_xo, int32_t G, void* stream);
int64_t dgppo_attn_xo_workspace_bytes(int32_t G);
int32_t dgppo_attn_bwd_xo_dw(const dgppo_env_cfg* cfg, int32_t F, int32_t H, int32_t Kp, const float* dzcat,
                             const float* attn, const float* qt, const float* Xa, const float* Xo_raw, const float* Wo,
                             int32_t ldwo, const float* bo, const float* efeat, float* dqt, float* dXa, float* dWo,
                             int32_t lddwo, float* dbo, float* workspace, int64_t workspace_bytes, int32_t G, void* stream);

int32_t dgppo_gnn_prep(const float* Wq, const float* bq, const float* Wk, const float* Wv, const float* bv,
                       const float* We, const float* Wu, float* Mcat, float* cvec, float* Wout, int32_t F, int32_t Fp,
                       int32_t D, int32_t H, int32_t Kp, void* stream);
int32_t dgppo_gnn_unprep(const float* dMcat, const float* dcvec, const float* dWout, const float* Wq, const float* bq,
                         const float* Wk, float* dWq, float* dbq, float* dWk, float* dWv, float* dbv, float* dWe,
                         float* dWu, int32_t F, int32_t Fp, int32_t D, int32_t H, int32_t Kp, void* stream);

int32_t dgppo_ln_relu_fwd(const float* x, const float* gamma, const float* beta, float* y, float* stats, int32_t M,
                          void* stream);
int32_t dgppo_ln_relu_bwd(const float* x, const float* y, const float* stats, const float* gamma, const float* dy,
                          float* dx, float* dgamma, float* dbeta, int32_t M, void* stream);

int32_t dgppo_gru_fwd(const float* gi, const float* Wh, const float* bhn, const float* h0, float* hs, float* hprev,
                      float* gates, int32_t n_seq, int32_t T, int32_t n_inner, void* stream);
int32_t dgppo_gru_fwd_h0_blocks(const float* gi, const float* Wh, const float* bhn, const float* h0,
                                int32_t rows_per_block, int64_t block_stride, float* hs, float* hprev, float* gates,
                                int32_t n_seq, int32_t T, int32_t n_inner, void* stream);
int32_t dgppo_gru_bwd(const float* dhs, const float* Wh, const float* hprev, const float* gates, float* dgi,
                      float* dgh, int32_t n_seq, int32_t T, int32_t n_inner, void* stream);
int32_t dgppo_gru_bwd_dhn(const float* dhs, const float* Wh, const float* hprev, const float* gates, float* dgi,
// ... 59 lines not shown
```

Before: 4.425 million.

## Fuse action sampling, env step, and next-step graph features into one lidar kernel

Adds a fused lidar wave kernel variant that samples or takes the mode of the tanh-normal action from the policy head output, steps the environment, and then writes the next step's node features, edge features, edge masks and the first GNN layer's dense projection. The rollout loop uses it by default when the config matches, so the separate feature-building and first dense-layer launches are skipped for every step after the first. The aim is to cut per-step kernel launches and global-memory round trips between the policy and the environment. In exchange, register and LDS pressure rise in the fused kernel, and ray constants are reloaded inside the loop.

```diff
diff --git a/dgppo_amd/csrc/env_step.h b/dgppo_amd/csrc/env_step.h
--- a/dgppo_amd/csrc/env_step.h
+++ b/dgppo_amd/csrc/env_step.h
@@ -23,6 +23,19 @@
   int B;
   float thr2_comm, thr2_lidar;
 };
+
+struct ActFeatArgs {
+  const float* ms;
+  const float* eps;
+  float* action;
+  float* log_pi;
+  int sample;
+  float *Xa, *Xo, *efeat, *emask;
+  const float *Mcat, *cvec;
+  float* qt0;
+  int max_blocks;
+};
+struct NoActFeat {};
 
 template <int SD>
 __device__ inline void state2feat(const float* s, float* f) {
@@ -160,3 +173,5 @@
 
 bool lidar_wave_has_instance(const dgppo_env_cfg& c);
 void launch_lidar_wave(const StepArgs& a, hipStream_t s);
+bool lidar_wave_has_act_instance(const dgppo_env_cfg& c);
+void launch_lidar_wave_act(const StepArgs& a, const ActFeatArgs& f, hipStream_t s);
diff --git a/dgppo_amd/csrc/env_step.hip b/dgppo_amd/csrc/env_step.hip
--- a/dgppo_amd/csrc/env_step.hip
+++ b/dgppo_amd/csrc/env_step.hip
@@ -716,6 +716,62 @@
                      gout, B, stream);
 }
 
+static bool act_step_ok(const dgppo_env_cfg& c, int Fp, int H) {
+  const bool lidar32 = cfg_is_lidar(c) && cfg_is_base_kind(c) && c.n_obs > 0 && c.n_rays == 32;
+  return lidar32 && c.top_k == 8 && c.eye_offset >= c.comm_radius && c.node_dim <= 8 && Fp == 8 && H == 3 && lidar_wave_has_act_instance(c);
+}
+
+extern "C" int32_t dgppo_env_act_step_feats_supported(const dgppo_env_cfg* cfg, int32_t Fp, int32_t H) {
+  if (!cfg || dgppo_validate_cfg(cfg) != 0 || cfg_is_vmas(*cfg)) return 0;
+  return act_step_ok(*cfg, Fp, H) ? 1 : 0;
+}
+
+extern "C" int32_t dgppo_env_act_step_feats(const dgppo_env_cfg* cfg, const float* agent, const float* goal, const float* obst,
+                                            const float* hits, const float* ray_cos, const float* ray_sin, const float* ms,
+                                            const float* eps, int32_t sample, float* action, float* log_pi, float* next_agent,
+                                            float* next_hits, float* reward, float* cost, float* Xa, float* Xo, float* efeat,
+                                            float* emask, int32_t Fp, const float* Mcat, const float* cvec, float* qt0, int32_t H,
+                                            int32_t max_blocks, int32_t B, void* stream) {
+  if (!cfg) { dgppo_set_error("cfg is NULL"); return -1; }
+  int32_t rc = dgppo_validate_cfg(cfg);
+  if (rc) return rc;
+  DGPPO_REFUSE_VMAS(cfg, "dgppo_env_act_step_feats", "dgppo_vmas_step");
+  DGPPO_REQUIRE(act_step_ok(*cfg, Fp, H), "env_act_step_feats: no kernel for this configuration, Fp=%d, H=%d (ask dgppo_env_act_step_feats_supported)", Fp, H);
+  DGPPO_REQUIRE(B >= 0 && max_blocks >= 0, "env_act_step_feats: B and max_blocks must be >= 0 (got %d, %d)", B, max_blocks);
+  if (B == 0) return 0;
+  DGPPO_REQUIRE(agent && goal && obst && hits && ray_cos && ray_sin, "env_act_step_feats: NULL state operand");
+  DGPPO_REQUIRE(ms && action && next_agent && next_hits && reward && cost, "env_act_step_feats: NULL operand");
+  DGPPO_REQUIRE(!sample || (eps && log_pi), "env_act_step_feats(sample): eps and log_pi must not be NULL");
+  DGPPO_REQUIRE(!Xa || (Xo && efeat && emask), "env_act_step_feats: Xa needs Xo, efeat and emask");
+  DGPPO_REQUIRE(!qt0 || (Mcat && cvec), "env_act_step_feats: qt0 needs Mcat and cvec");
+  auto al16 = [](const void* p) { return (((uintptr_t)p) & 15) == 0; };
+  DGPPO_REQUIRE(al16(agent) && al16(goal) && al16(obst) && al16(hits) && al16(next_agent) && al16(next_hits),
+                "env_act_step_feats: the record operands must be 16-byte aligned");
+  DGPPO_REQUIRE(al16(Xa) && al16(Xo) && al16(efeat) && al16(emask) && al16(qt0),
+                "env_act_step_feats: Xa, Xo, efeat, emask and qt0 must be 16-byte aligned");
+  DGPPO_REQUIRE((((uintptr_t)ms | (uintptr_t)eps | (uintptr_t)action | (uintptr_t)log_pi | (uintptr_t)Mcat | (uintptr_t)cvec) & 3) == 0,
+                "env_act_step_feats: operands must be 4-byte aligned");
+  StepArgs a;
+  a.cfg = *cfg;
+  a.agent = agent; a.action = nullptr; a.goal = goal; a.obst = obst; a.hits = hits;
+  a.ray_cos = ray_cos; a.ray_sin = ray_sin;
+  a.next_agent = next_agent; a.next_hits = next_hits; a.reward = reward; a.cost = cost;
+  a.has_graph = 0;
+  a.g = dgppo_graph_out{};
+  a.mode = MODE_STEP;
+  a.B = B;
+  a.rcp_n = fdiv_rcp(cfg->n_agents); a.rcp_k = fdiv_rcp(cfg->top_k); a.rcp_no = fdiv_rcp(cfg->n_obs);
+  a.rcp_no4 = fdiv_rcp(4 * cfg->n_obs);
+  a.thr2_comm = sqrt_threshold(cfg->comm_radius);
+  a.thr2_lidar = sqrt_threshold(cfg->lidar_mask_radius);
+  ActFeatArgs f;
+  f.ms = ms; f.eps = eps; f.action = action; f.log_pi = log_pi; f.sample = sample ? 1 : 0;
+  f.Xa = Xa; f.Xo = Xo; f.efeat = efeat; f.emask = emask; f.Mcat = Mcat; f.cvec = cvec; f.qt0 = qt0; f.max_blocks = max_blocks;
+  launch_lidar_wave_act(a, f, (hipStream_t)stream);
+  DGPPO_LAUNCH_CHECK();
+  return 0;
+}
+
 extern "C" int32_t dgppo_graph_materialize(const dgppo_env_cfg* cfg, const float* agent, const float* goal,
                                            const float* obst, const float* hits, const dgppo_graph_out* gout, int32_t B,
                                            void* stream) {
diff --git a/dgppo_amd/csrc/env_wave.hip b/dgppo_amd/csrc/env_wave.hip
--- a/dgppo_amd/csrc/env_wave.hip
+++ b/dgppo_amd/csrc/env_wave.hip
@@ -1,4 +1,6 @@
 #include "env_step.h"
+#include "nn_head.h"
+#include <type_traits>
 
 #ifndef DGPPO_WAVE_WPE
 #define DGPPO_WAVE_WPE 5
@@ -85,6 +87,13 @@
   float nodes[GRAPH ? ceil4(C::N * C::ND) : 4];
 };
 
+constexpr int ACT_FP = 8, ACT_H = 3, ACT_HF = ACT_H * ACT_FP;
+constexpr int ACT_MAX_NA = 8;
+template <int SD, bool SPREAD, int NA, int NO>
+struct alignas(16) WaveLdsAct : WaveLds<SD, SPREAD, NA, NO, false> {
+  float mc[ACT_FP * ACT_HF + ACT_HF];
+};
+
 __device__ inline float raw_min(float a, float b) { float r; asm("v_min_f32 %0, %1, %2" : "=v"(r) : "v"(a), "v"(b)); return r; }
 __device__ inline float raw_max(float a, float b) { float r; asm("v_max_f32 %0, %1, %2" : "=v"(r) : "v"(a), "v"(b)); return r; }
 
@@ -121,10 +130,12 @@
   return x;
 }
 
-template <int SD, bool SPREAD, int NA, int NO, int WPB, int MODE, bool GRAPH>
-__global__ void __launch_bounds__(WPB * 64) __attribute__((amdgpu_waves_per_eu(GRAPH ? DGPPO_WAVE_WPE : DGPPO_WAVE_WPE_COMPACT, 8))) lidar_wave_kernel(StepArgs a) {
+template <int SD, bool SPREAD, int NA, int NO, int WPB, int MODE, bool GRAPH, bool FUSE = false>
+__global__ void __launch_bounds__(WPB * 64) __attribute__((amdgpu_waves_per_eu((GRAPH || FUSE) ? DGPPO_WAVE_WPE : DGPPO_WAVE_WPE_COMPACT, 8)))
+lidar_wave_kernel(StepArgs a, std::conditional_t<FUSE, ActFeatArgs, NoActFeat> f) {
+  static_assert(!FUSE || (MODE == MODE_STEP && !GRAPH), "the act-step form is a compact step");
   using C = WC<SD, SPREAD, NA, NO>;
-  using LT = WaveLds<SD, SPREAD, NA, NO, GRAPH>;
+  using LT = std::conditional_t<FUSE, WaveLdsAct<SD, SPREAD, NA, NO>, WaveLds<SD, SPREAD, NA, NO, GRAPH>>;
   constexpr int K = C::K, ND = C::ND, N = C::N, PAD = C::PAD, NIT = C::NIT, GS = C::GS, E = C::E;
   extern __shared__ float4 smem4[];
   int lane = threadIdx.x & 63;
@@ -139,21 +150,21 @@
   constexpr bool do_sense = (MODE != MODE_GRAPH);
   constexpr bool has_graph = GRAPH;
   const float sr = c.comm_radius;
-  const int r = lane & 31;
-  const int hi_half = lane >> 5;
-  const float cr = do_sense ? a.ray_cos[r] : 0.0f, sn = do_sense ? a.ray_sin[r] : 0.0f;
-  const uint32_t below = (1u << r) - 1u;
+  const int r0 = lane & 31;
+  const int hi_half0 = lane >> 5;
+  const float cr0 = (do_sense && !FUSE) ? a.ray_cos[r0] : 0.0f, sn0 = (do_sense && !FUSE) ? a.ray_sin[r0] : 0.0f;
+  const uint32_t below0 = (1u << r0) - 1u;
 
   constexpr int I_AG = NA * SD / 4, I_OB = NO * 4, I_HI = (MODE != MODE_SENSE) ? NA * K * 2 / 4 : 0,
-                I_AC = (MODE == MODE_STEP) ? NA * 2 / 4 : 0;
+                I_AC = (MODE == MODE_STEP && !FUSE) ? NA * 2 / 4 : 0;
   constexpr int IT = 2 * I_AG + I_OB + I_HI + I_AC, NSLOT = (IT + 63) / 64;
   static_assert(MODE != MODE_STEP || (NA * 2) % 4 == 0, "the action block is staged as float4");
   const char* gsrc[NSLOT];
   uint32_t gstride[NSLOT];
   float4 pf[NSLOT];
-#pragma unroll
-  for (int j = 0; j < NSLOT; ++j) {
-    const int q = j * 64 + lane;
+  struct StageSrc { const char* p; uint32_t stride; };
+  auto stage_src = [&](int ln, int j) -> StageSrc {
+    const int q = j * 64 + ln;
     const char* base = reinterpret_cast<const char*>(a.agent);
     uint32_t stride = NA * SD * 4;
     int q0 = 0;
@@ -161,9 +172,15 @@
     if (q >= 2 * I_AG) { base = reinterpret_cast<const char*>(a.obst); stride = NO * 64; q0 = 2 * I_AG; }
     if (I_HI > 0 && q >= 2 * I_AG + I_OB) { base = reinterpret_cast<const char*>(a.hits); stride = NA * K * 8; q0 = 2 * I_AG + I_OB; }
     if (I_AC > 0 && q >= 2 * I_AG + I_OB + I_HI) { base = reinterpret_cast<const char*>(a.action); stride = NA * 8; q0 = 2 * I_AG + I_OB + I_HI; }
-    gsrc[j] = base + (q - q0) * 16;
-    gstride[j] = stride;
+    return StageSrc{base + (q - q0) * 16, stride};
+  };
+#pragma unroll
+  for (int j = 0; j < NSLOT; ++j) {
+    const StageSrc ss = stage_src(lane, j);
+    gsrc[j] = ss.p;
+    gstride[j] = ss.stride;
   }
+  static_assert(!FUSE || (2 * NA <= 64 && ND <= ACT_FP), "one lane per action component; node rows fit Fp = 8");
   {
     const int b0 = blockIdx.x * WPB + wave;
     if (b0 < a.B) {
@@ -171,6 +188,10 @@
       for (int j = 0; j < NSLOT; ++j)
         if (j * 64 + lane < IT) pf[j] = *reinterpret_cast<const float4*>(gsrc[j] + (size_t)b0 * gstride[j]);
     }
+  }
+  if constexpr (FUSE) {
+    if (f.qt0 != nullptr)
+      for (int i = lane; i < ACT_FP * ACT_HF + ACT_HF; i += 64) L.mc[i] = (i < ACT_FP * ACT_HF) ? f.Mcat[i] : f.cvec[i - ACT_FP * ACT_HF];
   }
   if (has_graph)
     for (int i = lane; i < ceil4(N * ND) / 4; i += 64) reinterpret_cast<float4*>(L.nodes)[i] = make_float4(0.0f, 0.0f, 0.0f, 0.0f);
@@ -182,21 +203,53 @@
 
   for (int b = blockIdx.x * WPB + wave; b < a.B; b += gridDim.x * WPB) {
     asm volatile("" : "+v"(lane));
+    const int r = FUSE ? (lane & 31) : r0;
+    const int hi_half = FUSE ? (lane >> 5) : hi_half0;
+    const float cr = FUSE ? a.ray_cos[lane & 31] : cr0, sn = FUSE ? a.ray_sin[lane & 31] : sn0;
+    const uint32_t below = FUSE ? ((1u << (lane & 31)) - 1u) : below0;
 #ifdef DGPPO_STAMPS
     const bool stamp_on = (b == 0);
     if ((threadIdx.x & 63) == 0 && gw < 8192 && b == gw) g_wspan[3 * gw + 1] = __builtin_amdgcn_s_memtime();
     if (blockIdx.x == 0 && threadIdx.x == 0 && stamp_on) g_wstamps[40] = __builtin_amdgcn_s_memrealtime();
 #endif
     PHASE("P0_stage", 0);
+    float h_mu = 0.0f, h_st = 0.0f, h_eps = 0.0f;
+    if constexpr (FUSE) {
+      if (lane < 2 * NA) {
+        const float* m = f.ms + ((size_t)b * NA + (lane >> 1)) * 4 + (lane & 1);
+        h_mu = m[0];
+        if (f.sample) { h_st = m[2]; h_eps = f.eps[(size_t)b * NA * 2 + lane]; }
+      }
+    }
 #pragma unroll
     for (int j = 0; j < NSLOT; ++j)
       if (j * 64 + lane < IT) reinterpret_cast<float4*>(L.agent)[j * 64 + lane] = pf[j];
+    if constexpr (FUSE) {
+      if (lane < 2 * NA) {
+        float act, lp = 0.0f;
+        if (f.sample) {
+          const float sd = tn_std(h_st);
+          act = tn_sample_dim(h_mu, sd, h_eps);
+          lp = tn_log_prob_dim(act, h_mu, sd);
+        } else {
+          act = tn_mode_dim(h_mu);
+        }
+        L.act[lane] = act;
+        f.action[(size_t)b * NA * 2 + lane] = act;
+        if (f.sample) {
+          const float lp1 = dpp<DPP_XOR1>(lp);
+          if ((lane & 1) == 0) f.log_pi[(size_t)b * NA + (lane >> 1)] = lp + lp1;
+        }
+      }
+    }
     {
       const int bn = b + gridDim.x * WPB;
       if (bn < a.B) {
 #pragma unroll
-        for (int j = 0; j < NSLOT; ++j)
-          if (j * 64 + lane < IT) pf[j] = *reinterpret_cast<const float4*>(gsrc[j] + (size_t)bn * gstride[j]);
+        for (int j = 0; j < NSLOT; ++j) {
+          const StageSrc ss = FUSE ? stage_src(lane, j) : StageSrc{gsrc[j], gstride[j]};
+          if (j * 64 + lane < IT) pf[j] = *reinterpret_cast<const float4*>(ss.p + (size_t)bn * ss.stride);
+        }
       }
     }
     WSYNC();
@@ -358,6 +411,47 @@
     if (a.next_agent != nullptr) {
       float4* o4 = reinterpret_cast<float4*>(a.next_agent + (size_t)b * NA * SD);
       for (int i = lane; i < NA * SD / 4; i += 64) o4[i] = reinterpret_cast<const float4*>(L.next)[i];
+    }
+    if constexpr (FUSE) {
+      if (f.Xa != nullptr) {
+#pragma unroll
+        for (int q0 = 0; q0 < 4 * NA; q0 += 64) {
+          const int q = q0 + lane;
+          if (q < 4 * NA) {
+            const int nd = q >> 1, col0 = (q & 1) * 4;
+            const bool is_goal = nd >= NA;
+            const float* src = is_goal ? L.goal + (nd - NA) * SD : L.next + nd * SD;
+            const int one = is_goal ? SD + 1 : SD + 2;
+            float v[4];
+#pragma unroll
+            for (int k = 0; k < 4; ++k) {
+              const int col = col0 + k;
+              v[k] = (col < SD) ? src[col < SD ? col : 0] : ((col == one) ? 1.0f : 0.0f);
+            }
+            float* dst = is_goal ? f.Xo + ((size_t)b * (NA + NA * K) + (nd - NA)) * ACT_FP + col0
+                                 : f.Xa + ((size_t)b * NA + nd) * ACT_FP + col0;
+            *reinterpret_cast<float4*>(dst) = make_float4(v[0], v[1], v[2], v[3]);
+          }
+        }
+      }
+      if (f.qt0 != nullptr) {
+        constexpr int NQ = ACT_HF / 4;
+#pragma unroll
+        for (int q0 = 0; q0 < NA * NQ; q0 += 64) {
+          const int q = q0 + lane;
+          if (q < NA * NQ) {
+            const int row = q / NQ, c0 = (q - row * NQ) * 4;
+            float4 acc = *reinterpret_cast<const float4*>(L.mc + ACT_FP * ACT_HF + c0);
+#pragma unroll
+            for (int k = 0; k < ACT_FP; ++k) {
+              const float xv = (k < SD) ? L.next[row * SD + (k < SD ? k : 0)] : ((k == SD + 2) ? 1.0f : 0.0f);
+              const float4 w = *reinterpret_cast<const float4*>(L.mc + k * ACT_HF + c0);
+              acc.x = fmaf(xv, w.x, acc.x); acc.y = fmaf(xv, w.y, acc.y); acc.z = fmaf(xv, w.z, acc.z); acc.w = fmaf(xv, w.w, acc.w);
+            }
+            *reinterpret_cast<float4*>(f.qt0 + ((size_t)b * NA + row) * ACT_HF + c0) = acc;
+          }
+        }
+      }
     }
     if (has_graph) {
       for (int q = lane; q < NA * SD; q += 64) {
@@ -722,6 +816,62 @@
       float4* o4 = reinterpret_cast<float4*>(a.next_hits + (size_t)b * NA * K * 2);
       for (int i = lane; i < NA * K * 2 / 4; i += 64) o4[i] = reinterpret_cast<const float4*>(L.hits)[i];
     }
+    if constexpr (FUSE) {
+      if (f.Xa != nullptr) {
+#pragma unroll
+        for (int q0 = 0; q0 < 2 * NA * K; q0 += 64) {
+          const int q = q0 + lane;
+          if (q < 2 * NA * K) {
+            const int h = q >> 1, col0 = (q & 1) * 4;
+            float v[4];
+#pragma unroll
+            for (int k = 0; k < 4; ++k) {
+              const int col = col0 + k;
+              v[k] = (col < 2) ? L.hits[h * 2 + (col < 2 ? col : 0)] : ((col == SD) ? 1.0f : 0.0f);
+            }
+            *reinterpret_cast<float4*>(f.Xo + ((size_t)b * (NA + NA * K) + NA + h) * ACT_FP + col0) = make_float4(v[0], v[1], v[2], v[3]);
+          }
+        }
+        constexpr int S = NA + GS + K, NE = NA * S;
+        static_assert(NE % 4 == 0, "masks leave as float4");
+#pragma unroll
+        for (int base = 0; base < NE; base += 64) {
+          const int idx = base + lane;
+          bool mask = false;
+          if (idx < NE) {
+            const int i = idx / S, s = idx - i * S;
+            const float4 fi = reinterpret_cast<const float4*>(fa_ptr)[i];
+            const float px = L.next[i * SD], py = L.next[i * SD + 1];
+            float4 e;
+            if (s < NA) {
+              const float4 fj = reinterpret_cast<const float4*>(fa_ptr)[s];
+              e = make_float4(fi.x - fj.x, fi.y - fj.y, fi.z - fj.z, fi.w - fj.w);
+              const float dx = px - L.next[s * SD], dy = py - L.next[s * SD + 1];
+              mask = (i != s) && (dx * dx + dy * dy < a.thr2_comm);
+            } else if (s < NA + GS) {
+              const int gi = SPREAD ? (s - NA) : i;
+              const float4 fg = reinterpret_cast<const float4*>(fg_ptr)[gi];
+              e = make_float4(fi.x - fg.x, fi.y - fg.y, fi.z - fg.z, fi.w - fg.w);
+              mask = true;
+            } else {
+              const int m = s - NA - GS;
+              const float lx = px - L.hits[(i * K + m) * 2], ly = py - L.hits[(i * K + m) * 2 + 1];
+              e = make_float4(lx, ly, 0.0f, 0.0f);
+              mask = lx * lx + ly * ly < a.thr2_lidar;
+            }
+            reinterpret_cast<float4*>(f.efeat)[(size_t)b * NE + idx] = e;
+          }
+          const unsigned long long bits = __builtin_amdgcn_ballot_w64(mask);
+          const int i4 = base + 4 * lane;
+          if (lane < 16 && i4 < NE) {
+            const unsigned mb = (unsigned)(bits >> (4 * lane));
+            *reinterpret_cast<float4*>(f.emask + (size_t)b * NE + i4) =
+                make_float4((mb & 1u) ? 1.0f : 0.0f, (mb & 2u) ? 1.0f : 0.0f, (mb & 4u) ? 1.0f : 0.0f, (mb & 8u) ? 1.0f : 0.0f);
+          }
+        }
+      }
+      WSYNC();
+    }
     if (!has_graph) continue;
     PHASE("P5_graph", 8);
     {
@@ -811,11 +961,32 @@
   int blocks = (a.B + WPB - 1) / WPB;
   if (blocks > max_blocks) blocks = max_blocks;
   const dim3 g(blocks), t(WPB * 64);
-#define LAUNCH(M_, G_) hipLaunchKernelGGL((lidar_wave_kernel<SD, SPREAD, NA, NO, WPB, M_, G_>), g, t, (G_) ? smem_g : smem_c, s, a)
+#define LAUNCH(M_, G_) hipLaunchKernelGGL((lidar_wave_kernel<SD, SPREAD, NA, NO, WPB, M_, G_>), g, t, (G_) ? smem_g : smem_c, s, a, NoActFeat{})
   if (a.mode == MODE_STEP) { if (a.has_graph) LAUNCH(MODE_STEP, true); else LAUNCH(MODE_STEP, false); }
   else if (a.mode == MODE_SENSE) { if (a.has_graph) LAUNCH(MODE_SENSE, true); else LAUNCH(MODE_SENSE, false); }
   else LAUNCH(MODE_GRAPH, true);
 #undef LAUNCH
+}
+
+template <int SD, bool SPREAD, int NA, int NO>
+void launch_inst_act(const StepArgs& a, const ActFeatArgs& f, hipStream_t s) {
+  constexpr size_t per_wave_g = sizeof(WaveLds<SD, SPREAD, NA, NO, true>);
+  constexpr int WPB = (per_wave_g * 4 <= 40 * 1024) ? 4 : ((per_wave_g * 2 <= 52 * 1024) ? 2 : 1);
+  constexpr size_t smem = sizeof(WaveLdsAct<SD, SPREAD, NA, NO>) * WPB;
+  static_assert(smem <= 64 * 1024, "LDS slab too large");
+  auto kern = lidar_wave_kernel<SD, SPREAD, NA, NO, WPB, MODE_STEP, false, true>;
+  static int per_cu = 0, n_cu = 0;
+  if (per_cu == 0) {
+    int n = 0;
+    per_cu = (hipOccupancyMaxActiveBlocksPerMultiprocessor(&n, kern, WPB * 64, smem) == hipSuccess && n > 0) ? n : 1;
+    int dev = 0, v = 0;
+    n_cu = (hipGetDevice(&dev) == hipSuccess && hipDeviceGetAttribute(&v, hipDeviceAttributeMultiprocessorCount, dev) == hipSuccess && v > 0) ? v : 256;
+  }
+  int max_blocks = n_cu * per_cu;
+  if (f.max_blocks > 0 && f.max_blocks < max_blocks) max_blocks = f.max_blocks;
+  int blocks = (a.B + WPB - 1) / WPB;
+  if (blocks > max_blocks) blocks = max_blocks;
+  hipLaunchKernelGGL(kern, dim3(blocks), dim3(WPB * 64), smem, s, a, f);
 }
 
 template <int SD_, bool SPREAD_, int NA_, int NO_>
@@ -849,6 +1020,14 @@
 #endif
 
 bool lidar_wave_has_instance(const dgppo_env_cfg& c) { return with_instance(c, [](auto) {}); }
+bool lidar_wave_has_act_instance(const dgppo_env_cfg& c) { return c.n_agents <= ACT_MAX_NA && lidar_wave_has_instance(c); }
+
+void launch_lidar_wave_act(const StepArgs& a, const ActFeatArgs& f, hipStream_t s) {
+  with_instance(a.cfg, [&](auto inst) {
+    using I = decltype(inst);
+    if constexpr (I::NA <= ACT_MAX_NA) launch_inst_act<I::SD, I::SPREAD, I::NA, I::NO>(a, f, s);
+  });
+}
 
 void launch_lidar_wave(const StepArgs& a, hipStream_t s) {
   with_instance(a.cfg, [&](auto inst) {
diff --git a/dgppo_amd/csrc/nn_elem.hip b/dgppo_amd/csrc/nn_elem.hip
--- a/dgppo_amd/csrc/nn_elem.hip
+++ b/dgppo_amd/csrc/nn_elem.hip
@@ -498,27 +498,7 @@
   return gru_bwd_launch<true>(a, (hipStream_t)stream);
 }
 
-#define STD_INIT_INV (-0.43275212956718856f)
-#define STD_MIN 1e-5f
-#define THRESH 0.999f
-#define INV_THRESH 3.8002011672502f
-#define LOG_EPS (-6.907755278982137f)
-#define HALF_LOG_2PI 0.9189385332046727f
-#define LOG2_F 0.6931471805599453f
-
-__device__ inline float softplusf_(float x) { return (x > 20.0f) ? x : log1pf(expf(x)); }
-#define NDTR_SERIES_BELOW (-10.0f)
-__device__ inline float ndtr_tail_series(float z2) { return 1.0f - 1.0f / z2 + 3.0f / (z2 * z2) - 15.0f / (z2 * z2 * z2); }
-__device__ inline float log_ndtrf_(float z) {
-  if (z > NDTR_SERIES_BELOW) return logf(0.5f * erfcf(-z * 0.70710678118654752f));
-  const float z2 = z * z;
-  return -0.5f * z2 - logf(-z) - HALF_LOG_2PI + logf(ndtr_tail_series(z2));
-}
-__device__ inline float dlog_ndtrf_(float z) {
-  if (z > NDTR_SERIES_BELOW) return 0.3989422804014327f * expf(-0.5f * z * z) / (0.5f * erfcf(-z * 0.70710678118654752f));
-  return -z / ndtr_tail_series(z * z);
-}
-__device__ inline float tanh_fldj(float x) { return 2.0f * (LOG2_F - x - softplusf_(-2.0f * x)); }
+#include "nn_head.h"
 
 struct HeadArgs {
   const float* ms;
@@ -535,15 +515,6 @@
   float clip_eps, coef_ent, inv_count;
 };
 
-__device__ inline float tn_log_prob_dim(float act, float mu, float sd) {
-  const float ac = fminf(fmaxf(act, -THRESH), THRESH);
-  if (ac <= -THRESH) return log_ndtrf_((-INV_THRESH - mu) / sd) - LOG_EPS;
-  if (ac >= THRESH) return log_ndtrf_(-(INV_THRESH - mu) / sd) - LOG_EPS;
-  const float x = atanhf(ac);
-  const float z = (x - mu) / sd;
-  return -0.5f * z * z - logf(sd) - HALF_LOG_2PI - tanh_fldj(x);
-}
-
 __global__ void __launch_bounds__(256) policy_head_kernel(HeadArgs a) {
   float acc[4] = {0.0f, 0.0f, 0.0f, 0.0f};
   const int rows_pad = (a.rows + 255) & ~255;
@@ -554,17 +525,17 @@
   const float mu[2] = {m.x, m.y};
   const float st[2] = {m.z, m.w};
   float sd[2];
-  for (int d = 0; d < 2; ++d) sd[d] = softplusf_(st[d] + STD_INIT_INV) + STD_MIN;
+  for (int d = 0; d < 2; ++d) sd[d] = tn_std(st[d]);
   if (a.mode == 1) {
     if (valid) {
-      a.action[row * 2] = tanhf(mu[0]);
-      a.action[row * 2 + 1] = tanhf(mu[1]);
+      a.action[row * 2] = tn_mode_dim(mu[0]);
+      a.action[row * 2 + 1] = tn_mode_dim(mu[1]);
     }
     continue;
   }
   float act[2];
   if (a.mode == 0) {
-    for (int d = 0; d < 2; ++d) act[d] = tanhf(mu[d] + sd[d] * a.eps[row * 2 + d]);
+    for (int d = 0; d < 2; ++d) act[d] = tn_sample_dim(mu[d], sd[d], a.eps[row * 2 + d]);
     if (valid) {
       a.action[row * 2] = act[0];
       a.action[row * 2 + 1] = act[1];
diff --git a/dgppo_amd/csrc/nn_head.h b/dgppo_amd/csrc/nn_head.h
--- /dev/null
+++ b/dgppo_amd/csrc/nn_head.h
@@ -0,0 +1,58 @@
+#pragma once
+#include "common.h"
+
+#define STD_INIT_INV (-0.43275212956718856f)
+#define STD_MIN 1e-5f
+#define THRESH 0.999f
+#define INV_THRESH 3.8002011672502f
+#define LOG_EPS (-6.907755278982137f)
+#define HALF_LOG_2PI 0.9189385332046727f
+#define LOG2_F 0.6931471805599453f
+
+__device__ inline float softplusf_(float x) {
+#pragma clang fp contract(fast)
+  return (x > 20.0f) ? x : log1pf(__builtin_expf(x));
+}
+#define NDTR_SERIES_BELOW (-10.0f)
+__device__ inline float ndtr_tail_series(float z2) {
+#pragma clang fp contract(fast)
+  return 1.0f - 1.0f / z2 + 3.0f / (z2 * z2) - 15.0f / (z2 * z2 * z2);
+}
+__device__ inline float log_ndtrf_(float z) {
+#pragma clang fp contract(fast)
+  if (z > NDTR_SERIES_BELOW) return __builtin_logf(0.5f * erfcf(-z * 0.70710678118654752f));
+  const float z2 = z * z;
+  return -0.5f * z2 - __builtin_logf(-z) - HALF_LOG_2PI + __builtin_logf(ndtr_tail_series(z2));
+}
+__device__ inline float dlog_ndtrf_(float z) {
+#pragma clang fp contract(fast)
+  if (z > NDTR_SERIES_BELOW) return 0.3989422804014327f * __builtin_expf(-0.5f * z * z) / (0.5f * erfcf(-z * 0.70710678118654752f));
+  return -z / ndtr_tail_series(z * z);
+}
+__device__ inline float tanh_fldj(float x) {
+#pragma clang fp contract(fast)
+  return 2.0f * (LOG2_F - x - softplusf_(-2.0f * x));
+}
+
+__device__ inline float tn_log_prob_dim(float act, float mu, float sd) {
+#pragma clang fp contract(fast)
+  const float ac = fminf(fmaxf(act, -THRESH), THRESH);
+  if (ac <= -THRESH) return log_ndtrf_((-INV_THRESH - mu) / sd) - LOG_EPS;
+  if (ac >= THRESH) return log_ndtrf_(-(INV_THRESH - mu) / sd) - LOG_EPS;
+  const float x = atanhf(ac);
+  const float z = (x - mu) / sd;
+  return -0.5f * z * z - __builtin_logf(sd) - HALF_LOG_2PI - tanh_fldj(x);
+}
+
+__device__ inline float tn_std(float std_trans) {
+#pragma clang fp contract(fast)
+  return softplusf_(std_trans + STD_INIT_INV) + STD_MIN;
+}
+__device__ inline float tn_mode_dim(float mu) {
+#pragma clang fp contract(fast)
+  return tanhf(mu);
+}
+__device__ inline float tn_sample_dim(float mu, float sd, float eps) {
+#pragma clang fp contract(fast)
+  return tanhf(mu + sd * eps);
+}
diff --git a/dgppo_amd/engine.py b/dgppo_amd/engine.py
--- a/dgppo_amd/engine.py
+++ b/dgppo_amd/engine.py
@@ -110,13 +110,15 @@
 class Engine:
     def __init__(self, cfg: N.EnvCfg, hyper: Hyper, device, T: int = 128,
                  allreduce: Optional[Callable[[torch.Tensor], None]] = None, world: int = 1, prepass_graphs: int = 1 << 20,
-                 use_graphs: bool = False, multi_stream: bool = False, algo: str = "dgppo", rank: int = 0):
+                 use_graphs: bool = False, multi_stream: bool = False, algo: str = "dgppo", rank: int = 0,
+                 fused_step: bool = True):
         self.cfg, self.hp, self.device, self.T = cfg, hyper, device, T
         assert algo in ("dgppo", "informarl", "hcbfcrpo", "informarl_lagr"), algo
         self.algo = algo
         self.use_graphs = use_graphs and os.environ.get("DGPPO_HIPGRAPH", "1") != "0"
         self.multi_stream = multi_stream and os.environ.get("DGPPO_MULTI_STREAM", "1") != "0"
         self._side_streams = None
+        self.fused_step = bool(fused_step) and OE.act_step_feats_supported(cfg, nets.input_width(cfg), nets.H_HEADS)
         self._ro_cache: Dict[tuple, dict] = {}
         self._upd_graph: dict = {}
         self.n_cost = cfg.n_cost
@@ -229,6 +231,21 @@
     def _rollout_steps(self, ro: RolloutData, eps, B: int, stochastic: bool):
         cfg, T, n = self.cfg, self.T, self.cfg.n_agents
         tag = "ro" if stochastic else "rod"
+        if self.fused_step:
+            pol, R = self.policy, B * n
+            feats = self._feats(tag, ro.states_tm[0], B)
+            Mcat, cvec = pol.pp("gnn0.Mcat"), pol.pp("gnn0.cvec")
+            qt0 = pol.arena.get(f"{tag}.qt0", R, Mcat.shape[1])
+            K.dense_fwd(feats.Xa, Mcat, cvec, qt0)
+            for t in range(T):
+                act = pol.forward(feats, n_seq=R, T=1, h0=ro.rnn_tm[t].view(R, self.HC), tag=tag,
+                                  hs_out=ro.rnn_tm[t + 1].view(R, self.HC), train=False, qt0=qt0)
+                nxt = dict(Xa=feats.Xa, Xo=feats.Xo, efeat=feats.efeat, emask=feats.emask, Fp=feats.Fp, Mcat=Mcat, cvec=cvec,
+                           qt0=qt0, H=nets.H_HEADS) if t + 1 < T else {}
+                OE.act_step_feats(cfg, ro.states_tm[t], act["ms"], eps[t] if stochastic else None, ro.action_tm[t],
+                                  ro.log_pi_tm[t] if stochastic else None, ro.states_tm[t + 1], ro.reward_tm[t], ro.cost_tm[t],
+                                  **nxt)
+            return
         for t in range(T):
             feats = self._feats(tag, ro.states_tm[t], B)
             act = self.policy.forward(feats, n_seq=B * n, T=1, h0=ro.rnn_tm[t].view(B * n, self.HC), tag=tag,
diff --git a/dgppo_amd/nets.py b/dgppo_amd/nets.py
--- a/dgppo_amd/nets.py
+++ b/dgppo_amd/nets.py
@@ -231,7 +231,7 @@
         self.grads.zero_()
 
     def forward(self, feats: GraphFeats, n_seq: int, T: int, h0: Optional[torch.Tensor], tag: str = "f",
-                hs_out: Optional[torch.Tensor] = None, train: bool = True):
+                hs_out: Optional[torch.Tensor] = None, train: bool = True, qt0: Optional[torch.Tensor] = None):
         cfg, G, A = self.cfg, feats.G, self.arena
         n = cfg.n_agents
         R = G * n
@@ -240,8 +240,12 @@
         Xa, Xo = feats.Xa, feats.Xo
         xo_fused = None
         for l, (f, fp, d, kp) in enumerate(self.dims):
-            qt = A.get(f"{tag}.qt{l}", R, H_HEADS * fp)
-            K.dense_fwd(Xa, self.pp(f"gnn{l}.Mcat"), self.pp(f"gnn{l}.cvec"), qt)
+            if l == 0 and qt0 is not None:
+                assert tuple(qt0.shape) == (R, H_HEADS * fp), (tuple(qt0.shape), R, H_HEADS * fp)
+                qt = qt0
+            else:
+                qt = A.get(f"{tag}.qt{l}", R, H_HEADS * fp)
+                K.dense_fwd(Xa, self.pp(f"gnn{l}.Mcat"), self.pp(f"gnn{l}.cvec"), qt)
             zcat = A.get(f"{tag}.zcat{l}", R, kp)
             attn = A.get(f"{tag}.attn{l}", R, cfg.fan_in, H_HEADS) if train else None
             if xo_fused is not None:
diff --git a/dgppo_amd/ops_env.py b/dgppo_amd/ops_env.py
--- a/dgppo_amd/ops_env.py
+++ b/dgppo_amd/ops_env.py
@@ -253,6 +253,48 @@
              cost, graph)
 
 
+def act_step_feats_supported(cfg: N.EnvCfg, Fp: int, H: int) -> bool:
+    return bool(N.lib().dgppo_env_act_step_feats_supported(C.byref(cfg), C.c_int32(Fp), C.c_int32(H)))
+
+
+def act_step_feats(cfg: N.EnvCfg, st: State, ms, eps, action, log_pi, nst: State, reward, cost, Xa=None, Xo=None, efeat=None,
+                   emask=None, Fp: int = 8, Mcat=None, cvec=None, qt0=None, H: int = 3, max_blocks: int = 0):
+    s, e, ns = st.step, st.env, nst.step
+    agent = s["agent"]
+    B, n = agent.shape[0], cfg.n_agents
+    rc, rs = _rays(cfg, agent.device)
+    sample = eps is not None
+    N.expect_shape(ms, (B * n, 4), "ms")
+    N.expect_shape(action, (B, n, 2), "action")
+    N.expect_shape(ns["agent"], (B, n, cfg.state_dim), "next_agent")
+    N.expect_shape(ns["hits"], (B, n, cfg.top_k, 2), "next_hits")
+    N.expect_shape(reward, (B,), "reward")
+    N.expect_shape(cost, (B, n, cfg.n_cost), "cost")
+    if sample:
+        N.expect_shape(eps, (B * n, 2), "eps")
+        N.expect_shape(log_pi, (B, n), "log_pi")
+    if Xa is not None:
+        S = cfg.fan_in
+        N.expect_shape(Xa, (B * n, Fp), "Xa")
+        N.expect_shape(Xo, (B * (cfg.num_nodes - 1 - n), Fp), "Xo")
+        N.expect_shape(efeat, (B * n, S, 4), "efeat")
+        N.expect_shape(emask, (B * n, S), "emask")
+    if qt0 is not None:
+        N.expect_shape(Mcat, (Fp, H * Fp), "Mcat")
+        N.expect_shape(cvec, (H * Fp,), "cvec")
+        N.expect_shape(qt0, (B * n, H * Fp), "qt0")
+    rc_ = N.lib().dgppo_env_act_step_feats(
+        C.byref(cfg), N.ptr(agent, name="agent"), N.ptr(e["goal"], name="goal"), N.ptr(e.get("obst"), name="obst"),
+        N.ptr(s.get("hits"), name="hits"), N.ptr(rc, name="ray_cos"), N.ptr(rs, name="ray_sin"), N.ptr(ms, name="ms"),
+        N.ptr(eps, name="eps"), C.c_int32(1 if sample else 0), N.ptr(action, name="action"),
+        N.ptr(log_pi if sample else None, name="log_pi"), N.ptr(ns["agent"], name="next_agent"),
+        N.ptr(ns["hits"], name="next_hits"), N.ptr(reward, name="reward"), N.ptr(cost, name="cost"), N.ptr(Xa, name="Xa"),
+        N.ptr(Xo if Xa is not None else None, name="Xo"), N.ptr(efeat if Xa is not None else None, name="efeat"),
+        N.ptr(emask if Xa is not None else None, name="emask"), C.c_int32(Fp), N.ptr(Mcat, name="Mcat"),
+        N.ptr(cvec, name="cvec"), N.ptr(qt0, name="qt0"), C.c_int32(H), C.c_int32(max_blocks), C.c_int32(B), N.stream_ptr())
+    N.check(rc_, "dgppo_env_act_step_feats")
+
+
 def materialize(cfg: N.EnvCfg, st: State, graph: Dict[str, torch.Tensor]):
     if cfg.is_vmas:
         return vmas_graph_materialize(cfg, st.agent, st.body, st.scene, graph)
diff --git a/include/dgppo_hip.h b/include/dgppo_hip.h
--- a/include/dgppo_hip.h
+++ b/include/dgppo_hip.h
@@ -86,6 +86,14 @@
                        const float* ray_cos, const float* ray_sin,
                        float* next_agent, float* next_hits, float* reward, float* cost,
                        const dgppo_graph_out* gout, int32_t B, void* stream);
+
+int32_t dgppo_env_act_step_feats_supported(const dgppo_env_cfg* cfg, int32_t Fp, int32_t H);
+int32_t dgppo_env_act_step_feats(const dgppo_env_cfg* cfg, const float* agent, const float* goal, const float* obst,
+                                 const float* hits, const float* ray_cos, const float* ray_sin, const float* ms,
+                                 const float* eps, int32_t sample, float* action, float* log_pi, float* next_agent,
+                                 float* next_hits, float* reward, float* cost, float* Xa, float* Xo, float* efeat,
+                                 float* emask, int32_t Fp, const float* Mcat, const float* cvec, float* qt0, int32_t H,
+                                 int32_t max_blocks, int32_t B, void* stream);
 
 int32_t dgppo_graph_materialize(const dgppo_env_cfg* cfg,
                                 const float* agent, const float* goal,
```

Measured after the change: 4.515 million, median of 6. +2.0%, better.
